# marian42/shapegan

Measured on AMD Instinct MI355X. Metric: GAN train steps/sec @32^3 voxels (train_wgan.py 5 critic + 1 generator updates, batch 64/GPU), higher is better.
Workload: dtype f32; 1 GPU; train_wgan.py 32^3 voxel WGAN, fp32, batch=64 synthetic SDF grids (BASELINE configs[1]); global_batch=64, per_gpu_batch=64, parallelism=dp1

## Files before the change

shapegan_amd/csrc/conv3d.hip:

```cpp
#include "mfma_tile.h"
#include <stdlib.h>

#include "conv_common.h"
#include "../../include/shapegan_hip.h"

namespace sg {

struct PatchCtx {
    int base;
    int mask;
    __device__ __forceinline__ void set(const ConvGeom& g, uint32_t pos) {
        int n, od, oh, ow;
        decode_pos(g, pos, n, od, oh, ow);
        const int id0 = 2 * od - 1, ih0 = 2 * oh - 1, iw0 = 2 * ow - 1;
        base = n * g.Cx * g.ID * g.IH * g.IW + (id0 * g.IH + ih0) * g.IW + iw0;
        int m = 0;
#pragma unroll
        for (int t = 0; t < 4; ++t) {
            if ((unsigned)(id0 + t) < (unsigned)g.ID) m |= 1 << t;
            if ((unsigned)(ih0 + t) < (unsigned)g.IH) m |= 1 << (4 + t);
            if ((unsigned)(iw0 + t) < (unsigned)g.IW) m |= 1 << (8 + t);
        }
        mask = m;
    }
// ... 420 lines not shown
struct WgradEpi {
    float* dw;
    long ldw;
    struct Col {
        int j;
    };
    __device__ Col col(int j) const { return Col{j}; }
    __device__ void store(const Col& c, int i, int j, float v) const { dw[(long)i * ldw + c.j] = v; }
};

}

using namespace sg;

extern "C" {

static bool edge_enabled(int which = 7) {
    constexpr int off = SG_NO_EDGE;
    return (off & which) == 0;
}

size_t sg_conv3d_k4s2p1_dgrad_workspace_bytes(int Cout, int Cin) {
    const size_t a = (size_t)8 * Cout * 8 * Cin * sizeof(float), b = halo_dgrad_workspace_bytes(Cin, Cout);
    return a > b ? a : b;
}

size_t sg_conv3d_k4s2p1_dgrad_workspace_bytes_for(int batch, int Cin, int Cout, int OD, int OH, int OW) {
    const size_t a = sg_conv3d_k4s2p1_dgrad_workspace_bytes(Cout, Cin);
    const size_t b = (Cin == 1 && Cout <= 64) ? edge_dgrad_workspace_bytes(batch, OD, OH, OW) : 0;
    return a > b ? a : b;
}

size_t sg_conv3d_k4s2p1_wgrad_workspace_bytes(int batch, int Cin, int Cout, int OD, int OH, int OW) {
    const size_t a = (size_t)16 * Cout * Cin * 64 * sizeof(float);
    const size_t b = (Cin >= 2 && Cout >= 32) ? halo_wgrad_workspace_bytes(batch, Cin, Cout, OD, OH, OW) : 0;
    const size_t c = (Cin == 1 && Cout <= 64) ? edge_wgrad_workspace_bytes(batch, OD, OH, OW) : 0;
    const size_t ab = a > b ? a : b;
    return ab > c ? ab : c;
}

size_t sg_conv3d_k4s2p1_fwd_workspace_bytes(int batch, int Cin, int Cout, int OD, int OH, int OW) {
    const size_t per = (size_t)batch * Cout * OD * OH * OW;
    const size_t tiles = ((size_t)batch * OD * OH * OW + 63) / 64 * ((Cout + 63) / 64);
    const size_t splitk = tiles >= 512 ? 0 : per * 8 * sizeof(float);
    const size_t pack = halo_fwd_workspace_bytes(Cin, Cout);
    const size_t edge = (Cin == 1 && Cout <= 64) ? edge_fwd_workspace_bytes(batch, OD, OH, OW) : 0;
    const size_t sp = (OD == 4 && OH == 4 && OW == 4) ? pack + splitk : (splitk > pack ? splitk : pack);
    return sp > edge ? sp : edge;
}

static int check_sizes(const ConvGeom& g, int batch, const char* who) {
    const long npos = (long)batch * g.O3();
    if (npos >= (1L << 31) || (long)batch * g.Cx * g.I3() >= (1L << 31) || (long)batch * g.Cy * g.O3() >= (1L << 31))
        SG_FAIL(SG_ERR_ARG, "%s: tensors of 2^31 elements or more are not supported (32-bit gather offsets)", who);
    return 0;
}

}

static int fwd_call(const float* x, const float* w, const float* bias, float* y, int batch, int Cin, int Cin_total,
                    int Cx, int Cout, int ID, int IH, int IW, int act, float slope, void* workspace,
                    size_t workspace_bytes, hipStream_t stream, bool packed_already) {
    SG_CHECK_ARG(x && w && y && batch > 0 && Cin > 0 && Cin <= Cin_total && Cin <= Cx && Cout > 0);
    ConvGeom g;
    if (make_geom(g, ID, IH, IW, Cx, Cout)) SG_FAIL(SG_ERR_ARG, "sg_conv3d_k4s2p1_fwd: spatial dims must be even and >= 2");
    if (check_sizes(g, batch, "sg_conv3d_k4s2p1_fwd")) return SG_ERR_ARG;
    const long npos = (long)batch * g.O3();
    if (Cin == 1 && edge_enabled(1) &&
        edge_fwd_try(x, w, bias, y, batch, Cin, Cin_total, g, Cout, act, slope, workspace, workspace_bytes, stream) == 1) {
        SG_CHECK_LAUNCH();
        return SG_OK;
    }
    {
        const int rc = halo_fwd_try(x, w, bias, y, batch, Cin, Cin_total, g, Cout, act, slope, workspace, workspace_bytes,
                                    stream, 0, 0, packed_already);
        if (rc < 0) return rc;
        if (rc == 1) {
            SG_CHECK_LAUNCH();
            return SG_OK;
        }
        if (rc > 16) {
            const int csplit = rc - 16;
            FwdEpi epi{y, bias, g.O3(), Cout, FastDiv((uint32_t)g.O3()), act, slope};
            const float* partial = reinterpret_cast<const float*>(static_cast<const char*>(workspace) + halo_fwd_workspace_bytes(Cin, Cout));
            const long fb = (long)Cout * ((npos + 1023) >> 10);
            hipLaunchKernelGGL((splitk_finalize_kernel<FwdEpi>), dim3((unsigned)fb), dim3(256), 0, stream, partial, epi, Cout, (int)npos,
                               csplit);
            SG_CHECK_LAUNCH();
            return SG_OK;
        }
    }
    MatRowMajor la;
    la.p = w;
    la.ld = (long)Cin_total * 64;
    FwdPatchLoader lb;
    lb.x = x;
    lb.g = g;
    FwdEpi epi{y, bias, g.O3(), Cout, FastDiv((uint32_t)g.O3()), act, slope};
    size_t ws_use = workspace ? workspace_bytes : 0;
    const size_t ws_query = sg_conv3d_k4s2p1_fwd_workspace_bytes(batch, Cin, Cout, g.OD, g.OH, g.OW);
    if (ws_use > ws_query) ws_use = ws_query;
    launch_tile_gemm(la, lb, epi, Cout, (int)npos, Cin * 64, (float*)workspace, ws_use, stream);
    SG_CHECK_LAUNCH();
    return SG_OK;
}

extern "C" {

int sg_conv3d_k4s2p1_fwd(const float* x, const float* w, const float* bias, float* y, int batch, int Cin, int Cin_total,
                         int Cx, int Cout, int ID, int IH, int IW, int act, float slope, void* workspace,
                         size_t workspace_bytes, hipStream_t stream) {
    return fwd_call(x, w, bias, y, batch, Cin, Cin_total, Cx, Cout, ID, IH, IW, act, slope, workspace, workspace_bytes, stream, false);
}
int sg_conv3d_k4s2p1_fwd_keep(const float* x, const float* w, const float* bias, float* y, int batch, int Cin, int Cin_total,
                              int Cx, int Cout, int ID, int IH, int IW, int act, float slope, void* workspace,
                              size_t workspace_bytes, int weights_unchanged, hipStream_t stream) {
    return fwd_call(x, w, bias, y, batch, Cin, Cin_total, Cx, Cout, ID, IH, IW, act, slope, workspace, workspace_bytes, stream,
                    weights_unchanged != 0);
}

int sg_conv3d_k4s2p1_fwd_impl(const float* x, const float* w, const float* bias, float* y, int batch, int Cin,
                              int Cin_total, int Cx, int Cout, int ID, int IH, int IW, int act, float slope,
                              void* workspace, size_t workspace_bytes, int impl, int debug, hipStream_t stream) {
    SG_CHECK_ARG(x && w && y && batch > 0 && Cin > 0 && Cin <= Cin_total && Cin <= Cx && Cout > 0);
    ConvGeom g;
    if (make_geom(g, ID, IH, IW, Cx, Cout)) SG_FAIL(SG_ERR_ARG, "sg_conv3d_k4s2p1_fwd_impl: bad spatial dims");
    if (check_sizes(g, batch, "sg_conv3d_k4s2p1_fwd_impl")) return SG_ERR_ARG;
    if (impl == 1) {
        const int rc = halo_fwd_try(x, w, bias, y, batch, Cin, Cin_total, g, Cout, act, slope, workspace, workspace_bytes,
                                    stream, 1, debug);
        if (rc != 1) SG_FAIL(SG_ERR_ARG, "sg_conv3d_k4s2p1_fwd_impl: shape not eligible for the LDS-halo kernel");
        SG_CHECK_LAUNCH();
        return SG_OK;
    }
    const long npos = (long)batch * g.O3();
    MatRowMajor la;
    la.p = w;
    la.ld = (long)Cin_total * 64;
    FwdPatchLoader lb;
    lb.x = x;
    lb.g = g;
    FwdEpi epi{y, bias, g.O3(), Cout, FastDiv((uint32_t)g.O3()), act, slope};
    launch_tile_gemm(la, lb, epi, Cout, (int)npos, Cin * 64, (float*)workspace, workspace ? workspace_bytes : 0, stream);
    SG_CHECK_LAUNCH();
    return SG_OK;
}

}

static int dgrad_call(const float* dy, const float* w, const float* bias, float* dx, int batch, int Cin, int Cin_total, int Cx,
                      int Cout, int ID, int IH, int IW, int act, float slope, void* workspace, size_t workspace_bytes,
                      hipStream_t stream, bool packed_already) {
    SG_CHECK_ARG(dy && w && dx && batch > 0 && Cin > 0 && Cin <= Cin_total && Cin <= Cx && Cout > 0);
    ConvGeom g;
    if (make_geom(g, ID, IH, IW, Cx, Cout)) SG_FAIL(SG_ERR_ARG, "sg_conv3d_k4s2p1_dgrad: spatial dims must be even and >= 2");
    if (check_sizes(g, batch, "sg_conv3d_k4s2p1_dgrad")) return SG_ERR_ARG;
    const long npos = (long)batch * g.O3();
    if (Cin == 1 && edge_enabled(2) &&
        edge_dgrad_try(dy, w, bias, dx, batch, Cin, Cin_total, g, Cout, act, slope, workspace, workspace_bytes, stream) == 1) {
        SG_CHECK_LAUNCH();
        return SG_OK;
    }
    if (Cin == 1 && g.OD % kO1D == 0 && g.OH % kO1H == 0 && g.OW % kO1W == 0 && (long)g.Cy * g.O3() * 4 < (long)kBufRange) {
        const int ntd = g.OD / kO1D, nth = g.OH / kO1H, ntw = g.OW / kO1W;
        const size_t lds = (size_t)(2 * kO1CC * (kO1CH + 8) + 8) * sizeof(float);
        static SgPerDeviceOnce attr_once;
        if (attr_once.begin()) {
            (void)hipFuncSetAttribute(reinterpret_cast<const void*>(dgrad_out1_tile_kernel),
                                      hipFuncAttributeMaxDynamicSharedMemorySize, (int)lds);
            attr_once.end();
        }
        hipLaunchKernelGGL(dgrad_out1_tile_kernel, dim3((unsigned)((long)batch * ntd * nth * ntw)), dim3(256), lds, stream, dy, w,
                           bias, dx, g, Cout, Cin_total, ntd, nth, ntw, act, slope);
        SG_CHECK_LAUNCH();
        return SG_OK;
    }
    if (Cin == 1 && Cout <= 512) {
        hipLaunchKernelGGL(dgrad_out1_kernel, dim3((unsigned)((npos + 255) / 256)), dim3(256),
                           (size_t)Cout * 64 * sizeof(float), stream, dy, w, bias, dx, g, Cout, Cin_total, (int)npos, act,
                           slope);
        SG_CHECK_LAUNCH();
        return SG_OK;
    }
    {
        const int rc = halo_dgrad_try(dy, w, bias, dx, batch, Cin, Cin_total, g, Cout, act, slope, workspace,
                                      workspace_bytes, stream, 0, packed_already);
        if (rc < 0) return rc;
        if (rc == 1) {
            SG_CHECK_LAUNCH();
            return SG_OK;
        }
    }
    const size_t need = (size_t)8 * Cout * 8 * Cin * sizeof(float);
    if (!workspace || workspace_bytes < need)
        SG_FAIL(SG_ERR_WORKSPACE, "sg_conv3d_k4s2p1_dgrad: workspace too small (%zu < %zu)", workspace_bytes, need);
    float* wt = (float*)workspace;
    if (!packed_already) {
        const long total = 8L * Cout * 8 * Cin;
        int blocks = (int)((total + 255) / 256);
        if (blocks > 2048) blocks = 2048;
        hipLaunchKernelGGL(pack_dgrad_weights_kernel, dim3(blocks), dim3(256), 0, stream, w, wt, Cout, Cin_total, Cin);
    }
    DgradWeightLoader la;
    la.wt = wt;
    la.Cin = Cin;
    la.pstride = (long)Cout * 8 * Cin;
    DgradPatchLoader lb;
    lb.dy = dy;
    lb.g = g;
    DgradEpi epi{dx, bias, g, act, slope};
    const int M = Cin, N = (int)npos, K = Cout * 8;
    const TilePlan p = plan_tiles(M, N, K, 0, 8);
    dim3 grid(sg_cdiv(N, 64 * p.tn), sg_cdiv(M, 64 * p.tm), 8);
#define SG_DGRAD_LAUNCH(TM_, TN_)                                                                                     \
    hipLaunchKernelGGL((tile_gemm_kernel<TM_, TN_, DgradWeightLoader, DgradPatchLoader, DgradEpi>), grid, dim3(256), 0, \
                       stream, la, lb, epi, M, N, K, 0)
    if (p.tm == 2 && p.tn == 2)
        SG_DGRAD_LAUNCH(2, 2);
    else if (p.tm == 2)
        SG_DGRAD_LAUNCH(2, 1);
    else if (p.tn == 2)
        SG_DGRAD_LAUNCH(1, 2);
    else
        SG_DGRAD_LAUNCH(1, 1);
#undef SG_DGRAD_LAUNCH
    SG_CHECK_LAUNCH();
    return SG_OK;
}

extern "C" {

int sg_conv3d_k4s2p1_dgrad(const float* dy, const float* w, const float* bias, float* dx, int batch, int Cin,
                           int Cin_total, int Cx, int Cout, int ID, int IH, int IW, int act, float slope,
                           void* workspace, size_t workspace_bytes, hipStream_t stream) {
    return dgrad_call(dy, w, bias, dx, batch, Cin, Cin_total, Cx, Cout, ID, IH, IW, act, slope, workspace, workspace_bytes, stream,
                      false);
}
int sg_conv3d_k4s2p1_dgrad_keep(const float* dy, const float* w, const float* bias, float* dx, int batch, int Cin,
                                int Cin_total, int Cx, int Cout, int ID, int IH, int IW, int act, float slope,
                                void* workspace, size_t workspace_bytes, int weights_unchanged, hipStream_t stream) {
    return dgrad_call(dy, w, bias, dx, batch, Cin, Cin_total, Cx, Cout, ID, IH, IW, act, slope, workspace, workspace_bytes, stream,
                      weights_unchanged != 0);
}

int sg_conv3d_k4s2p1_pack_images(int n, const int* kinds, const float* const* weights, void* const* workspaces,
                                 const size_t* workspace_bytes, const int* dims, int* served, hipStream_t stream) {
    SG_CHECK_ARG(n > 0 && n <= 8 && kinds && weights && workspaces && workspace_bytes && dims && served);
    PackJobs jobs;
    static const float dummy = 0.f;
    for (int i = 0; i < n; ++i) {
        const int* d = dims + 8 * i;
        const int batch = d[0], Cin = d[1], Cin_total = d[2], Cx = d[3], Cout = d[4];
        served[i] = 0;
        SG_CHECK_ARG(weights[i] && batch > 0 && Cin > 0 && Cin <= Cin_total && Cin <= Cx && Cout > 0 && (kinds[i] == 0 || kinds[i] == 1));
        ConvGeom g;
        if (make_geom(g, d[5], d[6], d[7], Cx, Cout)) SG_FAIL(SG_ERR_ARG, "sg_conv3d_k4s2p1_pack_images: bad spatial dims");
        if (check_sizes(g, batch, "sg_conv3d_k4s2p1_pack_images")) return SG_ERR_ARG;
        if (Cin == 1) continue;
        int rc;
        if (kinds[i] == 0)
            rc = halo_fwd_try(&dummy, weights[i], nullptr, const_cast<float*>(&dummy), batch, Cin, Cin_total, g, Cout, SG_ACT_NONE, 0.f,
                              workspaces[i], workspace_bytes[i], stream, 0, 0, false, &jobs);
        else
            rc = halo_dgrad_try(&dummy, weights[i], nullptr, const_cast<float*>(&dummy), batch, Cin, Cin_total, g, Cout, SG_ACT_NONE, 0.f,
                                workspaces[i], workspace_bytes[i], stream, 0, false, &jobs);
        if (rc < 0) return rc;
        served[i] = rc == 1;
    }
    halo_pack_jobs_launch(jobs, stream);
    SG_CHECK_LAUNCH();
    return SG_OK;
}

long long sg_conv3d_k4s2p1_image_layout(int kind, const int* dims, size_t workspace_bytes) {
    if (!dims || (kind != 0 && kind != 1)) return 0;
    const int batch = dims[0], Cin = dims[1], Cin_total = dims[2], Cx = dims[3], Cout = dims[4];
    if (batch <= 0 || Cin <= 1 || Cin > Cin_total || Cin > Cx || Cout <= 0) return 0;
    ConvGeom g;
    if (make_geom(g, dims[5], dims[6], dims[7], Cx, Cout)) return 0;
    if ((long)batch * g.O3() >= (1L << 31) || (long)batch * g.I3() >= (1L << 31)) return 0;
    PackJobs jobs;
    static const float dummy = 0.f;
    char* const base = reinterpret_cast<char*>(uintptr_t(1) << 20);
    const int rc = kind == 0 ? halo_fwd_try(&dummy, &dummy, nullptr, const_cast<float*>(&dummy), batch, Cin, Cin_total, g, Cout, SG_ACT_NONE,
                                            0.f, base, workspace_bytes, nullptr, 0, 0, false, &jobs)
                             : halo_dgrad_try(&dummy, &dummy, nullptr, const_cast<float*>(&dummy), batch, Cin, Cin_total, g, Cout,
                                              SG_ACT_NONE, 0.f, base, workspace_bytes, nullptr, 0, false, &jobs);
    if (rc != 1 || jobs.n != 1) return 0;
    const PackJob& j = jobs.job[0];
    unsigned long long h = 1469598103934665603ull;
    const long long f[7] = {j.kind + 1, j.Cout, j.Cin_total, j.Cin, j.nt, (long long)(reinterpret_cast<char*>(j.wp) - base), 0x5347};
    for (long long v : f)
        for (int b = 0; b < 8; ++b) {
            h ^= (unsigned long long)(v >> (8 * b)) & 0xffull;
            h *= 1099511628211ull;
        }
    h &= 0x7fffffffffffffffull;
    return h ? (long long)h : 1;
}

int sg_conv3d_k4s2p1_dgrad_impl(const float* dy, const float* w, const float* bias, float* dx, int batch, int Cin,
                                int Cin_total, int Cx, int Cout, int ID, int IH, int IW, int act, float slope,
                                void* workspace, size_t workspace_bytes, int impl, hipStream_t stream) {
    SG_CHECK_ARG(dy && w && dx && batch > 0 && Cin > 0 && Cin <= Cin_total && Cin <= Cx && Cout > 0 && (impl & 1) &&
                 (impl == 1 || impl == 3 || impl == 9 || impl == 17 || impl == 33));
    ConvGeom g;
    if (make_geom(g, ID, IH, IW, Cx, Cout)) SG_FAIL(SG_ERR_ARG, "sg_conv3d_k4s2p1_dgrad_impl: bad spatial dims");
    if (check_sizes(g, batch, "sg_conv3d_k4s2p1_dgrad_impl")) return SG_ERR_ARG;
    const int rc = halo_dgrad_try(dy, w, bias, dx, batch, Cin, Cin_total, g, Cout, act, slope, workspace, workspace_bytes,
                                  stream, impl);
    if (rc != 1) SG_FAIL(SG_ERR_ARG, "sg_conv3d_k4s2p1_dgrad_impl: shape not eligible for the LDS-halo kernel");
    SG_CHECK_LAUNCH();
    return SG_OK;
}

int sg_conv3d_k4s2p1_wgrad_impl(const float* dy, const float* x, float* dw, int batch, int Cin, int Cin_total, int Cx,
                                int Cout, int ID, int IH, int IW, void* workspace, size_t workspace_bytes, int impl,
                                hipStream_t stream) {
    SG_CHECK_ARG(dy && x && dw && batch > 0 && Cin > 0 && Cin <= Cin_total && Cin <= Cx && Cout > 0 && impl == 1);
    ConvGeom g;
    if (make_geom(g, ID, IH, IW, Cx, Cout)) SG_FAIL(SG_ERR_ARG, "sg_conv3d_k4s2p1_wgrad_impl: bad spatial dims");
    if (check_sizes(g, batch, "sg_conv3d_k4s2p1_wgrad_impl")) return SG_ERR_ARG;
    const int rc = halo_wgrad_try(dy, x, dw, batch, Cin, Cin_total, g, Cout, workspace, workspace_bytes, stream, 1);
    if (rc != 1) SG_FAIL(SG_ERR_ARG, "sg_conv3d_k4s2p1_wgrad_impl: shape not eligible for the LDS-halo kernel");
    SG_CHECK_LAUNCH();
    return SG_OK;
}

int sg_conv3d_k4s2p1_wgrad_dy_image(int batch, int Cin, int Cout, int OD, int OH, int OW, size_t workspace_bytes, int* mt_total,
                                    long* nslice) {
    if (batch <= 0 || Cin <= 0 || Cout <= 0 || !mt_total || !nslice) return 0;
    ConvGeom g;
    if (make_geom(g, 2 * OD, 2 * OH, 2 * OW, Cin, Cout)) return 0;
    if (Cin == 1 && Cout <= 64) return 0;
    return halo_wgrad_dy_image_plan(batch, Cin, Cout, g, workspace_bytes, mt_total, nslice);
}
int sg_act_bwd_rowsum_pack8(const float* y, const float* dy, float* dz, float* rowsum, void* dz_image, long N, int C, long nslice,
                            int act, float slope, hipStream_t stream) {
    SG_CHECK_ARG(y && dy && dz && rowsum && dz_image && N > 0 && C > 0 && C % 128 == 0 && nslice == N * 8);
    SG_CHECK_ARG(act == SG_ACT_LEAKY || act == SG_ACT_RELU);
    SG_CHECK_ARG((((uintptr_t)y | (uintptr_t)dy | (uintptr_t)dz | (uintptr_t)dz_image) & 15) == 0);
    halo_act_bwd_pack8_launch(y, dy, dz, rowsum, dz_image, N * C, C, nslice, act, slope, stream);
    SG_CHECK_LAUNCH();
    return SG_OK;
}
int sg_conv3d_k4s2p1_wgrad_prepacked(const float* dy, const float* x, float* dw, int batch, int Cin, int Cin_total, int Cx,
                                     int Cout, int ID, int IH, int IW, void* workspace, size_t workspace_bytes, hipStream_t stream) {
    SG_CHECK_ARG(dy && x && dw && batch > 0 && Cin > 0 && Cin <= Cin_total && Cin <= Cx && Cout > 0);
    ConvGeom g;
    if (make_geom(g, ID, IH, IW, Cx, Cout)) SG_FAIL(SG_ERR_ARG, "sg_conv3d_k4s2p1_wgrad_prepacked: bad spatial dims");
    if (check_sizes(g, batch, "sg_conv3d_k4s2p1_wgrad_prepacked")) return SG_ERR_ARG;
    int mt;
    long ns;
    if (!halo_wgrad_dy_image_plan(batch, Cin, Cout, g, workspace_bytes, &mt, &ns))
        SG_FAIL(SG_ERR_ARG, "sg_conv3d_k4s2p1_wgrad_prepacked: this call is not served with a producer-written image");
    if (halo_wgrad_try(dy, x, dw, batch, Cin, Cin_total, g, Cout, workspace, workspace_bytes, stream, 0, true) != 1)
        SG_FAIL(SG_ERR_ARG, "sg_conv3d_k4s2p1_wgrad_prepacked: not served");
    SG_CHECK_LAUNCH();
    return SG_OK;
}

int sg_conv3d_k4s2p1_wgrad_act_eligible(int batch, int Cin, int Cout, int OD, int OH, int OW, int act) {
    const size_t x_bytes = ((size_t)batch * 8 * OD * OH * OW + (size_t)(2 * OH + 1) * 2 * OW + 4) * 4;
    const size_t dy_bytes = (size_t)batch * Cout * OD * OH * OW * 4;
    return Cin == 1 && Cout <= 64 && OW % 16 == 0 && (long)batch * OD * OH * OW >= 65536 && (act == SG_ACT_LEAKY || act == SG_ACT_RELU) &&
           x_bytes < (size_t)kBufRange && dy_bytes < (size_t)kBufRange && edge_enabled(4);
}
int sg_conv3d_k4s2p1_wgrad_act(const float* dy, const float* y, const float* x, float* dw, float* db, int batch, int Cin,
                               int Cin_total, int Cx, int Cout, int ID, int IH, int IW, int act, float slope, void* workspace,
                               size_t workspace_bytes, hipStream_t stream) {
    SG_CHECK_ARG(dy && y && x && dw && db && batch > 0 && Cin > 0 && Cin <= Cin_total && Cin <= Cx && Cout > 0);
    ConvGeom g;
    if (make_geom(g, ID, IH, IW, Cx, Cout)) SG_FAIL(SG_ERR_ARG, "sg_conv3d_k4s2p1_wgrad_act: spatial dims must be even and >= 2");
    if (check_sizes(g, batch, "sg_conv3d_k4s2p1_wgrad_act")) return SG_ERR_ARG;
    if (!sg_conv3d_k4s2p1_wgrad_act_eligible(batch, Cin, Cout, g.OD, g.OH, g.OW, act) ||
        edge_wgrad_try(dy, x, dw, batch, Cin, Cin_total, g, Cout, workspace, workspace ? workspace_bytes : 0, stream, 0, y, act, slope,
                       db) != 1)
        SG_FAIL(SG_ERR_ARG, "sg_conv3d_k4s2p1_wgrad_act: shape not served (see sg_conv3d_k4s2p1_wgrad_act_eligible) or workspace too small");
    SG_CHECK_LAUNCH();
    return SG_OK;
}

int sg_conv3d_k4s2p1_wgrad(const float* dy, const float* x, float* dw, int batch, int Cin, int Cin_total, int Cx,
                           int Cout, int ID, int IH, int IW, void* workspace, size_t workspace_bytes,
                           hipStream_t stream) {
    SG_CHECK_ARG(dy && x && dw && batch > 0 && Cin > 0 && Cin <= Cin_total && Cin <= Cx && Cout > 0);
    ConvGeom g;
    if (make_geom(g, ID, IH, IW, Cx, Cout)) SG_FAIL(SG_ERR_ARG, "sg_conv3d_k4s2p1_wgrad: spatial dims must be even and >= 2");
    if (check_sizes(g, batch, "sg_conv3d_k4s2p1_wgrad")) return SG_ERR_ARG;
    const long npos = (long)batch * g.O3();
    if (Cin == 1 && edge_enabled(4) &&
        edge_wgrad_try(dy, x, dw, batch, Cin, Cin_total, g, Cout, workspace, workspace ? workspace_bytes : 0, stream) == 1) {
        SG_CHECK_LAUNCH();
        return SG_OK;
    }
    {
        const int rc = halo_wgrad_try(dy, x, dw, batch, Cin, Cin_total, g, Cout, workspace, workspace ? workspace_bytes : 0,
                                      stream, 0);
        if (rc < 0) return rc;
        if (rc == 1) {
            SG_CHECK_LAUNCH();
            return SG_OK;
        }
    }
    WgradDyLoader la;
    la.dy = dy;
    la.O3 = (int)g.O3();
    la.Cy = Cout;
    la.dO3 = FastDiv((uint32_t)g.O3());
    WgradPatchLoader lb;
    lb.x = x;
    lb.g = g;
    WgradEpi epi{dw, (long)Cin_total * 64};
    launch_tile_gemm(la, lb, epi, Cout, Cin * 64, (int)npos, (float*)workspace, workspace ? workspace_bytes : 0, stream);
    SG_CHECK_LAUNCH();
    return SG_OK;
}

int sg_convT3d_k4s2p1_fwd(const float* x, const float* w, const float* bias, float* y, int batch, int Cin_T, int Cout_T,
                          int ID, int IH, int IW, int act, float slope, void* workspace, size_t workspace_bytes,
                          hipStream_t stream) {
    return sg_conv3d_k4s2p1_dgrad(x, w, bias, y, batch, Cout_T, Cout_T, Cout_T, Cin_T, 2 * ID, 2 * IH, 2 * IW, act,
                                  slope, workspace, workspace_bytes, stream);
}
int sg_convT3d_k4s2p1_to1_pre_eligible(int batch, int C, int ID, int IH, int IW) {
    return batch > 0 && C > 0 && C <= 64 && ID > 0 && IH > 0 && IW > 0 && IH * IW <= 256 &&
           (size_t)C * ID * IH * IW * 4 < (size_t)kBufRange && (long)batch * 8 * ID * IH * IW < (1L << 31);
}
static int convT_to1_pre(const float* x, const float* w, const float* bias, float* y, const float* in_scale,
                         const float* in_shift, int in_act, float in_slope, int batch, int C, int ID, int IH, int IW,
                         int act, float slope, int samples_per_group, long y_group_stride, int form, hipStream_t stream) {
    SG_CHECK_ARG(x && w && y && in_scale && in_shift && samples_per_group > 0 && batch % samples_per_group == 0 && form >= 0 && form <= 8);
    SG_CHECK_ARG(y_group_stride >= (long)samples_per_group * 8 * ID * IH * IW);
    if (!sg_convT3d_k4s2p1_to1_pre_eligible(batch, C, ID, IH, IW))
        SG_FAIL(SG_ERR_ARG, "sg_convT3d_k4s2p1_to1_pre: shape not served (C <= 64, IH * IW <= 256)");
    SG_CHECK_ARG(in_act == SG_ACT_NONE || in_act == SG_ACT_RELU || (in_act == SG_ACT_LEAKY && in_slope >= 0.f && in_slope <= 1.f));
    ConvGeom g;
    if (make_geom(g, 2 * ID, 2 * IH, 2 * IW, 1, C)) SG_FAIL(SG_ERR_ARG, "sg_convT3d_k4s2p1_to1_pre: bad spatial dims");
    if (edge_dgrad_stream_try(x, w, bias, y, batch, 1, 1, g, C, act, slope, stream, in_scale, in_shift, in_act, in_slope,
                              samples_per_group, y_group_stride, form) != 1)
        SG_FAIL(SG_ERR_ARG, "sg_convT3d_k4s2p1_to1_pre: not served");
    SG_CHECK_LAUNCH();
    return SG_OK;
}
int sg_convT3d_k4s2p1_to1_pre_grouped(const float* x, const float* w, const float* bias, float* y, const float* in_scale,
                                      const float* in_shift, int in_act, float in_slope, int batch, int C, int ID, int IH, int IW,
                                      int act, float slope, int samples_per_group, long y_group_stride, hipStream_t stream) {
    return convT_to1_pre(x, w, bias, y, in_scale, in_shift, in_act, in_slope, batch, C, ID, IH, IW, act, slope, samples_per_group,
                         y_group_stride, 0, stream);
}
int sg_convT3d_k4s2p1_to1_pre_impl(const float* x, const float* w, const float* bias, float* y, const float* in_scale,
                                   const float* in_shift, int in_act, float in_slope, int batch, int C, int ID, int IH, int IW,
                                   int act, float slope, int form, hipStream_t stream) {
    return convT_to1_pre(x, w, bias, y, in_scale, in_shift, in_act, in_slope, batch, C, ID, IH, IW, act, slope, batch,
                         (long)batch * 8 * ID * IH * IW, form, stream);
}
int sg_convT3d_k4s2p1_to1_pre(const float* x, const float* w, const float* bias, float* y, const float* in_scale,
                              const float* in_shift, int in_act, float in_slope, int batch, int C, int ID, int IH, int IW, int act,
                              float slope, hipStream_t stream) {
    return sg_convT3d_k4s2p1_to1_pre_grouped(x, w, bias, y, in_scale, in_shift, in_act, in_slope, batch, C, ID, IH, IW, act, slope,
                                             batch, (long)batch * 8 * ID * IH * IW, stream);
}
int sg_convT3d_k4s2p1_dgrad(const float* dy, const float* w, float* dx, int batch, int Cin_T, int Cout_T, int ID, int IH,
                            int IW, void* workspace, size_t workspace_bytes, hipStream_t stream) {
    return sg_conv3d_k4s2p1_fwd(dy, w, nullptr, dx, batch, Cout_T, Cout_T, Cout_T, Cin_T, 2 * ID, 2 * IH, 2 * IW,
                                SG_ACT_NONE, 0.f, workspace, workspace_bytes, stream);
}
int sg_convT3d_k4s2p1_wgrad(const float* dy, const float* x, float* dw, int batch, int Cin_T, int Cout_T, int ID, int IH,
                            int IW, void* workspace, size_t workspace_bytes, hipStream_t stream) {
    return sg_conv3d_k4s2p1_wgrad(x, dy, dw, batch, Cout_T, Cout_T, Cout_T, Cin_T, 2 * ID, 2 * IH, 2 * IW, workspace,
                                  workspace_bytes, stream);
}

}
```

shapegan_amd/csrc/conv3d_halo.hip:

```cpp
#include "conv_common.h"

#ifndef SG_RING
#define SG_RING 8
#endif
#ifndef SG_ABLATE
#define SG_ABLATE 0
#endif

namespace sg {

constexpr int kHD = 4, kHH = 18, kHWF = 18;
constexpr int kHWH = 10;
constexpr int kROWH = 2 * kHWH;
constexpr int kROWD = kHH * kROWH;
constexpr int kHS = kHD * kROWD;
constexpr int kCC = 4;

struct HaloFwdArgs {
    const float* x;
    const float4* wp;
    const float* bias;
    float* y;
    ConvGeom g;
    int Cin, Cout;
    int nth, ntw;
    FastDiv dntw, dnth, dOD;
    int act;
    float slope;
    int csplit;
    float* partial;
    long npos;
};

__global__ void __launch_bounds__(256) pack_fwd_weights_kernel(const float* __restrict__ w, float4* __restrict__ wp,
                                                               int Cout, int Cin_total, int Cin, int ntile) {
    const long G = (long)Cin * 8;
    const long total = (long)ntile * G * 64;
    for (long e = (long)blockIdx.x * 256 + threadIdx.x; e < total; e += (long)gridDim.x * 256) {
        const int lane = (int)(e & 63);
        const long q = e >> 6;
        const long g = q % G;
        const int mt = (int)(q / G);
        const int co = mt * 32 + (lane & 31);
        float4 v = make_float4(0.f, 0.f, 0.f, 0.f);
        if (co < Cout) {
            const float* src = w + (long)co * Cin_total * 64 + g * 8 + (lane >> 5);
            v = make_float4(src[0], src[2], src[4], src[6]);
        }
        wp[e] = v;
    }
}

template <int TN, int NW>
__global__ void __launch_bounds__(NW * 64) conv_fwd_halo_kernel(HaloFwdArgs a) {
    constexpr int kFR = NW * 2;
    constexpr int kNF = (kHD * kHH + kFR - 1) / kFR;
    constexpr int WN = 2 / TN;
    constexpr int ROWS = (NW / WN) * 32;
    constexpr int kRing = SG_RING;
    constexpr int kBUF = kCC * kHS;
    extern __shared__ __attribute__((aligned(16))) float halo[];
    lds_float* const hl = (lds_float*)halo;

    uint32_t twi, thi, od, n, q1, q2;
    a.dntw.divmod(blockIdx.x, q1, twi);
    a.dnth.divmod(q1, q2, thi);
    a.dOD.divmod(q2, n, od);
    const int oh0 = thi * 8, ow0 = twi * 8;
    const int co0 = blockIdx.y * ROWS;

    const int tid = threadIdx.x, lane = tid & 63;
    const int wave = __builtin_amdgcn_readfirstlane(tid >> 6);
    const int wm = wave / WN, wn = wave % WN, r = lane & 31, kpar = lane >> 5;
    const int lanebase = 2 * (wn * TN * 4 + (r >> 3)) * kROWH + kpar * kHWH + (r & 7);
    constexpr int kTNOFF = 2 * 4 * kROWH;

    f32x16 acc[TN];
#pragma unroll
    for (int u = 0; u < TN; ++u)
#pragma unroll
        for (int q = 0; q < 16; ++q) acc[u][q] = 0.f;

    const lds_float* bb[2][kCC][4];
#pragma unroll
    for (int b = 0; b < 2; ++b)
#pragma unroll
        for (int c = 0; c < kCC; ++c)
#pragma unroll
            for (int kd = 0; kd < 4; ++kd) {
                bb[b][c][kd] = hl + b * kBUF + c * kHS + kd * kROWD + lanebase;
                pin_vgpr(bb[b][c][kd]);
            }

    const int G = a.Cin * 8;
    const __amdgpu_buffer_rsrc_t wres = make_rsrc(a.wp + ((long)(co0 / 32 + wm) * G) * 64);
    const unsigned wvoff = lane * 16;

    const int I3 = a.g.ID * a.g.IH * a.g.IW;
    const __amdgpu_buffer_rsrc_t xres = make_rsrc(a.x + (long)n * a.g.Cx * I3);
    const int fl_w = tid & 31, frow = tid >> 5;
    const int iw = 2 * ow0 - 1 + fl_w;
    const bool wok = fl_w < kHWF && (unsigned)iw < (unsigned)a.g.IW;
    const int lds_w = (fl_w & 1) * kHWH + (fl_w >> 1);
    const int pad = (tid % (kHD * kHH * 2)) * kHWH + (kHWH - 1);
    unsigned goff[kNF];
    lds_float* sdst[kNF];
#pragma unroll
    for (int f = 0; f < kNF; ++f) {
        const int row = kFR * f + frow, hd = row / kHH, hh = row - hd * kHH;
        const int id = 2 * (int)od - 1 + hd, ih = 2 * oh0 - 1 + hh;
        const bool inbox = fl_w < kHWF && row < kHD * kHH;
        const bool ok = inbox && wok && (unsigned)id < (unsigned)a.g.ID && (unsigned)ih < (unsigned)a.g.IH;
        goff[f] = ok ? (unsigned)((id * a.g.IH + ih) * a.g.IW + iw) * 4u : kBufOutside;
        sdst[f] = hl + (inbox ? hd * kROWD + hh * kROWH + lds_w : pad);
        pin_vgpr(goff[f]);
        pin_vgpr(sdst[f]);
    }
    float fv[kCC][kNF];
    const unsigned chan_bytes = (unsigned)I3 * 4u;

#pragma unroll
    for (int c = 0; c < kCC; ++c)
#pragma unroll
        for (int f = 0; f < kNF; ++f) fv[c][f] = buf_load(xres, goff[f], c * chan_bytes);
    float4 aring[kRing];
#pragma unroll
    for (int u = 0; u < kRing; ++u) aring[u] = buf_load4(wres, wvoff, (unsigned)(u < G ? u : G - 1) * 1024u);
#pragma unroll
    for (int c = 0; c < kCC; ++c)
#pragma unroll
        for (int f = 0; f < kNF; ++f) sdst[f][c * kHS] = fv[c][f];
    __syncthreads();

    const int nstage = a.Cin / kCC;
    int gbase = kRing;

    auto stage = [&](auto tag, int s) {
        constexpr int CUR = decltype(tag)::value, NXT = CUR ^ 1;
        int cnext = (s + 1) * kCC;
        cnext = cnext > a.Cin - kCC ? a.Cin - kCC : cnext;
        const unsigned xs = (unsigned)cnext * chan_bytes;
        float bq[TN][4];
#pragma unroll
        for (int u = 0; u < TN; ++u) {
            const lds_float* hb = bb[CUR][0][0] + u * kTNOFF;
            bq[u][0] = hb[0];
            bq[u][1] = hb[1];
            bq[u][2] = hb[kROWH];
            bq[u][3] = hb[kROWH + 1];
        }
        __builtin_amdgcn_sched_barrier(0);
#pragma unroll
        for (int ci = 0; ci < kCC; ++ci) {
#pragma unroll
            for (int j = 0; j < 8; ++j) {
                const float4 a_cur = aring[(ci * 8 + j) % kRing];
                int gi = gbase + ci * 8 + j;
                gi = gi < G ? gi : G - 1;
                if (!(SG_ABLATE & 4)) aring[(ci * 8 + j) % kRing] = buf_load4(wres, wvoff, (unsigned)gi * 1024u);
                {
                    constexpr int NE = kCC * kNF;
                    const int gidx = ci * 8 + j;
#pragma unroll
                    for (int e = 0; e < NE; ++e) {
                        const int c = e / kNF, f = e % kNF;
                        if (e * 24 / NE + 8 == gidx && !(SG_ABLATE & 2)) sdst[f][NXT * kBUF + c * kHS] = fv[c][f];
                        if (e * 24 / NE == gidx && !(SG_ABLATE & 3)) fv[c][f] = buf_load(xres, goff[f], xs + c * chan_bytes);
                    }
                }
                float b[TN][4];
#pragma unroll
                for (int u = 0; u < TN; ++u)
#pragma unroll
                    for (int k = 0; k < 4; ++k) b[u][k] = bq[u][k];
                if (!(ci == kCC - 1 && j == 7) && !(SG_ABLATE & 16)) {
                    const int jn = (j + 1) & 7, cin = ci + ((j + 1) >> 3);
                    const lds_float* hb = bb[CUR][cin][jn >> 1] + (2 * (jn & 1)) * kROWH;
#pragma unroll
                    for (int u = 0; u < TN; ++u) {
                        bq[u][0] = hb[u * kTNOFF];
                        bq[u][1] = hb[u * kTNOFF + 1];
                        bq[u][2] = hb[u * kTNOFF + kROWH];
                        bq[u][3] = hb[u * kTNOFF + kROWH + 1];
                    }
                }
                __builtin_amdgcn_sched_barrier(0);
#pragma unroll
                for (int k = 0; k < 4; ++k)
#pragma unroll
                    for (int u = 0; u < TN; ++u) {
                        const float av = k == 0 ? a_cur.x : (k == 1 ? a_cur.y : (k == 2 ? a_cur.z : a_cur.w));
                        acc[u] = __builtin_amdgcn_mfma_f32_32x32x2f32(av, b[u][k], acc[u], 0, 0, 0);
                    }
                __builtin_amdgcn_sched_barrier(0);
            }
        }
        gbase += 8 * kCC;
        __syncthreads();
    };
    for (int s = 0; s + 1 < nstage; s += 2) {
        stage(IntTag<0>(), s);
        stage(IntTag<1>(), s + 1);
    }
    if (nstage & 1) stage(IntTag<0>(), nstage - 1);

    const long O3 = (long)a.g.OD * a.g.OH * a.g.OW;
    float bv[16];
#pragma unroll
    for (int q = 0; q < 16; ++q) {
        const int co = co0 + wm * 32 + (q & 3) + 8 * (q >> 2) + 4 * kpar;
        bv[q] = a.bias ? a.bias[co < a.Cout ? co : a.Cout - 1] : 0.f;
    }
#pragma unroll
    for (int u = 0; u < TN; ++u) {
        const int ph = (wn * TN + u) * 4 + (r >> 3), pw = r & 7;
        float* yo = a.y + (long)n * a.Cout * O3 + ((long)od * a.g.OH + (oh0 + ph)) * a.g.OW + (ow0 + pw);
#pragma unroll
        for (int q = 0; q < 16; ++q) {
            const int co = co0 + wm * 32 + (q & 3) + 8 * (q >> 2) + 4 * kpar;
            if (co < a.Cout) yo[(long)co * O3] = sg_apply_act(acc[u][q] + bv[q], a.act, a.slope);
        }
    }
}

constexpr int k4HALF = 5, k4ROW = 10, k4PLANE = 104, k4CH = 10 * k4PLANE;
constexpr int k4CC = 8;
constexpr int k4BUF = k4CC * k4CH;

__global__ void __launch_bounds__(512) conv_fwd_halo4_kernel(HaloFwdArgs a) {
    constexpr int kRing = 8;
    extern __shared__ __attribute__((aligned(16))) float halo[];
    lds_float* const hl = (lds_float*)halo;
    const int n = blockIdx.x, co0 = blockIdx.y * 64;
    const int cpw = a.Cin / a.csplit, cb = blockIdx.z * cpw;
    const int tid = threadIdx.x, lane = tid & 63;
    const int wave = __builtin_amdgcn_readfirstlane(tid >> 6);
    const int kh = wave >> 2, wm = (wave >> 1) & 1, wn = wave & 1, r = lane & 31, kpar = lane >> 5;
    const int p = wn * 32 + r, od = p >> 4, oh = (p >> 2) & 3, ow = p & 3;
    const int lanebase = 2 * od * k4PLANE + 2 * oh * k4ROW + kpar * k4HALF + ow;

    f32x16 acc;
#pragma unroll
    for (int q = 0; q < 16; ++q) acc[q] = 0.f;

    for (int e = tid; e < 2 * k4BUF; e += 512) hl[e] = 0.f;

    const lds_float* bb[2][4][4];
#pragma unroll
    for (int b = 0; b < 2; ++b)
#pragma unroll
        for (int c = 0; c < 4; ++c)
#pragma unroll
            for (int kd = 0; kd < 4; ++kd) {
                bb[b][c][kd] = hl + b * k4BUF + (kh * 4 + c) * k4CH + kd * k4PLANE + lanebase;
                pin_vgpr(bb[b][c][kd]);
            }
    const int G = a.Cin * 8;
    const __amdgpu_buffer_rsrc_t wres = make_rsrc(a.wp + ((long)(co0 / 32 + wm) * G) * 64);
    const unsigned wvoff = lane * 16;

    const int I3 = 512;
    const __amdgpu_buffer_rsrc_t xres = make_rsrc(a.x + ((long)n * a.g.Cx + cb) * I3);
    unsigned xvoff = tid * 4;
    lds_float* sdst = hl + ((tid >> 6) + 1) * k4PLANE + (((tid >> 3) & 7) + 1) * k4ROW + (((tid & 7) + 1) & 1) * k4HALF +
                      (((tid & 7) + 1) >> 1);
    pin_vgpr(xvoff);
    pin_vgpr(sdst);
    float fv[k4CC];
    __syncthreads();
#pragma unroll
    for (int c = 0; c < k4CC; ++c) fv[c] = buf_load(xres, xvoff, c * (I3 * 4));
    const int nstage = cpw / k4CC, nq = nstage * 32, s0 = cb / k4CC;
    auto group_of = [&](int q) {
        q = q < nq ? q : nq - 1;
        return ((q >> 5) + s0) * 64 + kh * 32 + (q & 31);
    };
    float4 aring[kRing];
#pragma unroll
    for (int u = 0; u < kRing; ++u) aring[u] = buf_load4(wres, wvoff, (unsigned)group_of(u) * 1024u);
#pragma unroll
    for (int c = 0; c < k4CC; ++c) sdst[c * k4CH] = fv[c];
    __syncthreads();

    int qbase = kRing;
    auto stage = [&](auto tag, int s) {
        constexpr int CUR = decltype(tag)::value, NXT = CUR ^ 1;
        int cnext = (s + 1) * k4CC;
        cnext = cnext > cpw - k4CC ? cpw - k4CC : cnext;
        const unsigned xs = (unsigned)cnext * (I3 * 4);
        float bq[4];
        {
            const lds_float* hb = bb[CUR][0][0];
            bq[0] = hb[0];
            bq[1] = hb[1];
            bq[2] = hb[k4ROW];
            bq[3] = hb[k4ROW + 1];
        }
        __builtin_amdgcn_sched_barrier(0);
#pragma unroll
        for (int ci = 0; ci < 4; ++ci) {
#pragma unroll
            for (int j = 0; j < 8; ++j) {
                const int gidx = ci * 8 + j;
                const float4 a_cur = aring[gidx % kRing];
                aring[gidx % kRing] = buf_load4(wres, wvoff, (unsigned)group_of(qbase + gidx) * 1024u);
#pragma unroll
                for (int c = 0; c < k4CC; ++c) {
                    if (2 * c + 8 == gidx) sdst[NXT * k4BUF + c * k4CH] = fv[c];
                    if (2 * c == gidx) fv[c] = buf_load(xres, xvoff, xs + c * (I3 * 4));
                }
                float b[4];
#pragma unroll
                for (int k = 0; k < 4; ++k) b[k] = bq[k];
                if (gidx + 1 < 32) {
                    const int jn = (j + 1) & 7, cin = ci + ((j + 1) >> 3);
                    const lds_float* hb = bb[CUR][cin][jn >> 1] + (2 * (jn & 1)) * k4ROW;
                    bq[0] = hb[0];
                    bq[1] = hb[1];
                    bq[2] = hb[k4ROW];
                    bq[3] = hb[k4ROW + 1];
                }
                __builtin_amdgcn_sched_barrier(0);
                acc = __builtin_amdgcn_mfma_f32_32x32x2f32(a_cur.x, b[0], acc, 0, 0, 0);
                acc = __builtin_amdgcn_mfma_f32_32x32x2f32(a_cur.y, b[1], acc, 0, 0, 0);
                acc = __builtin_amdgcn_mfma_f32_32x32x2f32(a_cur.z, b[2], acc, 0, 0, 0);
                acc = __builtin_amdgcn_mfma_f32_32x32x2f32(a_cur.w, b[3], acc, 0, 0, 0);
                __builtin_amdgcn_sched_barrier(0);
            }
        }
        qbase += 32;
        __syncthreads();
    };
    for (int s = 0; s + 1 < nstage; s += 2) {
        stage(IntTag<0>(), s);
        stage(IntTag<1>(), s + 1);
    }
    if (nstage & 1) stage(IntTag<0>(), nstage - 1);

    float* red = halo + ((wave & 3) * 16) * 64;
    if (kh == 1) {
#pragma unroll
        for (int q = 0; q < 16; ++q) red[q * 64 + lane] = acc[q];
    }
    __syncthreads();
    if (kh == 1) return;
    if (a.csplit > 1) {
        float* po = a.partial + (long)blockIdx.z * a.Cout * a.npos + (long)n * 64 + p;
#pragma unroll
        for (int q = 0; q < 16; ++q) {
            const int co = co0 + wm * 32 + (q & 3) + 8 * (q >> 2) + 4 * kpar;
            if (co < a.Cout) po[(long)co * a.npos] = acc[q] + red[q * 64 + lane];
        }
        return;
    }
    float* yo = a.y + (long)n * a.Cout * 64 + p;
#pragma unroll
    for (int q = 0; q < 16; ++q) {
        const int co = co0 + wm * 32 + (q & 3) + 8 * (q >> 2) + 4 * kpar;
        if (co < a.Cout) {
            const float bv = a.bias ? a.bias[co] : 0.f;
            yo[(long)co * 64] = sg_apply_act(acc[q] + red[q * 64 + lane] + bv, a.act, a.slope);
        }
    }
}

size_t halo_fwd_workspace_bytes(int Cin, int Cout) { return (size_t)((Cout + 127) / 128) * 128 * Cin * 64 * sizeof(float); }

int halo_fwd_try(const float* x, const float* w, const float* bias, float* y, int batch, int Cin, int Cin_total,
                 const ConvGeom& g, int Cout, int act, float slope, void* workspace, size_t workspace_bytes,
                 hipStream_t stream, int force, int debug, bool packed_already, PackJobs* collect) {
    if (g.OD == 4 && g.OH == 4 && g.OW == 4) {
        if (Cin % k4CC != 0 || Cin < 2 * k4CC || Cout < 32) return 0;
        if (!workspace || workspace_bytes < halo_fwd_workspace_bytes(Cin, Cout)) return 0;
        if ((long)g.Cx * 512 * 4 >= (long)kBufRange || (long)Cin * 8 * 1024 >= (long)kBufRange || batch > 65535 * 16) return 0;
        const int mtiles = sg_cdiv(Cout, 64);
        int csplit = 1;
        if (!force && (long)batch * mtiles < 160) {
            while (csplit < 8 && (long)batch * mtiles * csplit < 256 && (Cin / (2 * csplit)) % k4CC == 0 && Cin / (2 * csplit) >= 2 * k4CC)
                csplit *= 2;
            if (csplit == 1) return 0;
            if (workspace_bytes < halo_fwd_workspace_bytes(Cin, Cout) + (size_t)csplit * Cout * batch * 64 * sizeof(float)) return 0;
        }
        float4* wp = (float4*)workspace;
        const int ntile = mtiles * 2;
        const long total = (long)ntile * Cin * 8 * 64;
        int blocks = (int)((total + 255) / 256);
        if (blocks > 4096) blocks = 4096;
        if (collect) return collect->add(0, w, wp, Cout, Cin_total, Cin, ntile);
        if (!packed_already)
            hipLaunchKernelGGL(pack_fwd_weights_kernel, dim3(blocks), dim3(256), 0, stream, w, wp, Cout, Cin_total, Cin, ntile);
        HaloFwdArgs a;
        a.x = x;
        a.wp = wp;
        a.bias = bias;
        a.y = y;
        a.g = g;
        a.Cin = Cin;
        a.Cout = Cout;
        a.nth = a.ntw = 1;
        a.dntw = a.dnth = a.dOD = FastDiv(1);
        a.act = act;
        a.slope = slope;
        a.csplit = csplit;
        a.partial = reinterpret_cast<float*>(static_cast<char*>(workspace) + halo_fwd_workspace_bytes(Cin, Cout));
        a.npos = (long)batch * 64;
        const size_t lds4 = (size_t)2 * k4BUF * sizeof(float);
        static SgPerDeviceOnce attr_once;
        if (attr_once.begin()) {
            (void)hipFuncSetAttribute(reinterpret_cast<const void*>(conv_fwd_halo4_kernel),
                                      hipFuncAttributeMaxDynamicSharedMemorySize, (int)lds4);
            attr_once.end();
        }
        hipLaunchKernelGGL(conv_fwd_halo4_kernel, dim3((unsigned)batch, mtiles, csplit), dim3(512), lds4, stream, a);
        return csplit > 1 ? 16 + csplit : 1;
    }
    if (g.OW % 8 != 0 || g.OH % 8 != 0 || Cin % kCC != 0 || Cin < 8 || Cout < 32) return 0;
    if ((long)g.Cx * g.ID * g.IH * g.IW * 4 >= (long)kBufRange || (long)Cin * 8 * 1024 >= (long)kBufRange) return 0;
    if (!workspace || workspace_bytes < halo_fwd_workspace_bytes(Cin, Cout)) return 0;
    if ((long)batch * g.Cx * g.ID * g.IH * g.IW >= (1L << 31)) return 0;
    int variant = (debug >> 4) & 3;
    int rows = (Cout > 64 && ((debug >> 4) & 3) != 3) ? 128 : 64;
    const int ntw = g.OW / 8, nth = g.OH / 8;
    const long tiles = (long)batch * g.OD * nth * ntw;
    if (rows == 128 && variant == 0 && !(debug & 128)) {
        const long w128 = tiles * sg_cdiv(Cout, 128);
        if (w128 <= 128 || (w128 > 256 && w128 <= 384)) rows = 64;
    }
    const int mtiles = sg_cdiv(Cout, rows);
    if (!force && tiles * mtiles < (rows == 128 ? 144 : 192)) return 0;
    if (tiles >= (1L << 31)) return 0;
    if (variant == 0) variant = 2;
    size_t lds = (size_t)2 * kCC * kHS * sizeof(float);
    if (tiles * mtiles < 256 * 3 * 4 && !(debug & 64) && lds < 56 * 1024) lds = 56 * 1024;

    float4* wp = (float4*)workspace;
    {
        const int ntile = mtiles * rows / 32;
        const long total = (long)ntile * Cin * 8 * 64;
        int blocks = (int)((total + 255) / 256);
        if (blocks > 4096) blocks = 4096;
        if (collect) return collect->add(0, w, wp, Cout, Cin_total, Cin, ntile);
        if (!packed_already)
            hipLaunchKernelGGL(pack_fwd_weights_kernel, dim3(blocks), dim3(256), 0, stream, w, wp, Cout, Cin_total, Cin, ntile);
    }
    HaloFwdArgs a;
    a.x = x;
    a.wp = wp;
    a.bias = bias;
    a.y = y;
    a.g = g;
    a.Cin = Cin;
    a.Cout = Cout;
    a.nth = nth;
    a.ntw = ntw;
    a.dntw = FastDiv(ntw);
    a.dnth = FastDiv(nth);
    a.dOD = FastDiv(g.OD);
    a.act = act;
    a.slope = slope;
    dim3 grid((unsigned)tiles, mtiles);
    if (rows == 128 && variant == 2)
        hipLaunchKernelGGL((conv_fwd_halo_kernel<1, 8>), grid, dim3(512), lds, stream, a);
    else if (rows == 128)
        hipLaunchKernelGGL((conv_fwd_halo_kernel<2, 4>), grid, dim3(256), lds, stream, a);
    else
        hipLaunchKernelGGL((conv_fwd_halo_kernel<1, 4>), grid, dim3(256), lds, stream, a);
    return 1;
}


template <int MODE>
struct DBox;
template <>
struct DBox<0> {
    static constexpr int BH = 9, BW = 9, PL = 81, CH = 243, TNOFF = 36, WNOFF = 81;
};
template <>
struct DBox<1> {
    static constexpr int BH = 5, BW = 5, PL = 25, CH = 250, TNOFF = 50, WNOFF = 125;
};

struct HaloDgradArgs {
    const float* dy;
    const float4* wp;
    const float* bias;
    float* dx;
    ConvGeom g;
    int Cin, Cout, mtiles, batch;
    int ppw;
    FastDiv dntw, dnth, dntd;
    int act;
    float slope;
};

__global__ void __launch_bounds__(256) pack_dgrad_frag_kernel(const float* __restrict__ w, float4* __restrict__ wp,
                                                              int Cout, int Cin_total, int Cin, int MT) {
    const long total = 8L * MT * Cout * 64;
    for (long e = (long)blockIdx.x * 256 + threadIdx.x; e < total; e += (long)gridDim.x * 256) {
        const int lane = (int)(e & 63);
        long q = e >> 6;
        const int co = (int)(q % Cout);
        q /= Cout;
        const int mt = (int)(q % MT);
        const int p = (int)(q / MT);
        const int ci = mt * 32 + (lane & 31);
        float v[4] = {0.f, 0.f, 0.f, 0.f};
        if (ci < Cin) {
            const float* src = w + ((long)co * Cin_total + ci) * 64;
#pragma unroll
            for (int j = 0; j < 4; ++j) {
                const int t = 2 * j + (lane >> 5);
                const int kd = 1 - ((p >> 2) & 1) + 2 * ((t >> 2) & 1);
                const int kh = 1 - ((p >> 1) & 1) + 2 * ((t >> 1) & 1);
                const int kw = 1 - (p & 1) + 2 * (t & 1);
                v[j] = src[kd * 16 + kh * 4 + kw];
            }
        }
        wp[e] = make_float4(v[0], v[1], v[2], v[3]);
    }
}

__global__ void __launch_bounds__(256) pack_images_kernel(PackJobs jobs) {
    const PackJob& j = jobs.job[blockIdx.y];
    float4* __restrict__ wp = j.wp;
    const float* __restrict__ w = j.w;
    if (j.kind == 0) {
        const long G = (long)j.Cin * 8;
        const long total = (long)j.nt * G * 64;
        for (long e = (long)blockIdx.x * 256 + threadIdx.x; e < total; e += (long)gridDim.x * 256) {
            const int lane = (int)(e & 63);
            const long q = e >> 6;
            const long g = q % G;
            const int mt = (int)(q / G);
            const int co = mt * 32 + (lane & 31);
            float4 v = make_float4(0.f, 0.f, 0.f, 0.f);
            if (co < j.Cout) {
                const float* src = w + (long)co * j.Cin_total * 64 + g * 8 + (lane >> 5);
                v = make_float4(src[0], src[2], src[4], src[6]);
            }
            wp[e] = v;
        }
    } else {
        const int MT = j.nt;
        const long total = 8L * MT * j.Cout * 64;
        for (long e = (long)blockIdx.x * 256 + threadIdx.x; e < total; e += (long)gridDim.x * 256) {
            const int lane = (int)(e & 63);
            long q = e >> 6;
            const int co = (int)(q % j.Cout);
            q /= j.Cout;
            const int mt = (int)(q % MT);
            const int p = (int)(q / MT);
            const int ci = mt * 32 + (lane & 31);
            float v[4] = {0.f, 0.f, 0.f, 0.f};
            if (ci < j.Cin) {
                const float* src = w + ((long)co * j.Cin_total + ci) * 64;
#pragma unroll
                for (int jj = 0; jj < 4; ++jj) {
                    const int t = 2 * jj + (lane >> 5);
                    const int kd = 1 - ((p >> 2) & 1) + 2 * ((t >> 2) & 1);
                    const int kh = 1 - ((p >> 1) & 1) + 2 * ((t >> 1) & 1);
                    const int kw = 1 - (p & 1) + 2 * (t & 1);
                    v[jj] = src[kd * 16 + kh * 4 + kw];
                }
            }
            wp[e] = make_float4(v[0], v[1], v[2], v[3]);
        }
    }
}
int halo_pack_jobs_launch(const PackJobs& jobs, hipStream_t stream) {
    if (jobs.n <= 0) return 0;
    hipLaunchKernelGGL(pack_images_kernel, dim3(1024, jobs.n), dim3(256), 0, stream, jobs);
    return jobs.n;
}

template <int MODE, bool R32>
__device__ __forceinline__ void conv_dgrad_halo_body(HaloDgradArgs a) {
    constexpr int NTN = R32 ? 1 : 2;
    constexpr int kDCC = 16, kDNF = 16, kDBUF = kDNF * 256;
    using BX = DBox<MODE>;
    constexpr int kDB = BX::CH;
    extern __shared__ __attribute__((aligned(16))) float box[];
    uint32_t twi = 0, thi = 0, tdi = 0, n, q1, q2;
    if (MODE == 0) {
        a.dntw.divmod(blockIdx.x, q1, twi);
        a.dnth.divmod(q1, q2, thi);
        a.dntd.divmod(q2, n, tdi);
    } else {
        n = blockIdx.x * 2;
    }
    const int qd0 = tdi * 2, qh0 = thi * 8, qw0 = twi * 8;
    const int ci0 = blockIdx.y * (R32 ? 32 : 64);

    const int tid = threadIdx.x, lane = tid & 63;
    const int wave = __builtin_amdgcn_readfirstlane(tid >> 6);
    const int wm = R32 ? 0 : wave >> 1, wn = wave & 1, r = lane & 31, kpar = lane >> 5;
    const int tnf = R32 ? wave >> 1 : 0;
    const int lpart = MODE == 0 ? (r >> 3) * BX::BW + (r & 7) : (r >> 4) * BX::PL + ((r >> 2) & 3) * BX::BW + (r & 3);
    const int lanebase = wn * BX::WNOFF + tnf * BX::TNOFF + lpart + 1 - kpar;

    f32x16 acc[NTN];
#pragma unroll
    for (int t = 0; t < NTN; ++t)
#pragma unroll
        for (int q = 0; q < 16; ++q) acc[t][q] = 0.f;

    lds_float* const bl = (lds_float*)box;
    const lds_float* bb[2][kDCC];
#pragma unroll
    for (int b = 0; b < 2; ++b)
#pragma unroll
        for (int c = 0; c < kDCC; ++c) {
            bb[b][c] = bl + b * kDBUF + c * kDB + lanebase;
            pin_vgpr(bb[b][c]);
        }
    lds_float* sdst = bl + tid;
    pin_vgpr(sdst);

    const int G = a.Cout;
    const int par0 = blockIdx.z * a.ppw, par_end = par0 + a.ppw;
    const unsigned par_bytes = (unsigned)(a.mtiles * 2) * (unsigned)G * 1024u;
    const __amdgpu_buffer_rsrc_t wres = make_rsrc(a.wp + ((long)(R32 ? blockIdx.y : blockIdx.y * 2 + wm) * G) * 64);
    const unsigned wvoff = lane * 16;

    const int O3 = a.g.OD * a.g.OH * a.g.OW;
    const int obias = (a.g.OH + 1) * a.g.OW + 1;
    const __amdgpu_buffer_rsrc_t dres = __builtin_amdgcn_make_buffer_rsrc(
        const_cast<float*>(a.dy + (long)n * a.g.Cy * O3 - obias), 0, 1 << 26, 0x00020000);
    const unsigned chan_bytes = (unsigned)O3 * 4u;
    unsigned gword[kDNF], goff[kDNF];
#pragma unroll
    for (int f = 0; f < kDNF; ++f) {
        const int e = tid + 256 * f;
        const int ci = e / kDB;
        int rem = e - ci * kDB, smp = 0;
        if (MODE == 1) {
            smp = rem / 125;
            rem -= smp * 125;
        }
        const int hd = rem / BX::PL, hh = (rem - hd * BX::PL) / BX::BW, hw = rem % BX::BW;
        const int od = qd0 - 1 + hd, oh = qh0 - 1 + hh, ow = qw0 - 1 + hw;
        const bool never = e >= kDCC * kDB || (int)n + smp >= a.batch;
        const unsigned cls = (od < 0 ? 1u << 26 : 0u) | (od + 1 >= a.g.OD ? 1u << 27 : 0u) | (oh < 0 ? 1u << 28 : 0u) |
                             (oh + 1 >= a.g.OH ? 1u << 29 : 0u) | (ow < 0 ? 1u << 30 : 0u) | (ow + 1 >= a.g.OW ? 1u << 31 : 0u);
        const int off0 = (smp * a.g.Cy + ci) * O3 + (od * a.g.OH + oh) * a.g.OW + ow + obias;
        gword[f] = never ? 0xffffffffu : ((unsigned)off0 * 4u) | cls;
        pin_vgpr(gword[f]);
    }
    unsigned pshift = 0;
    auto set_goff = [&](int par) __attribute__((always_inline)) {
        const int pd = (par >> 2) & 1, ph = (par >> 1) & 1, pw = par & 1;
        const unsigned mask = 0x03ffffffu | (pd ? 1u << 27 : 1u << 26) | (ph ? 1u << 29 : 1u << 28) | (pw ? 1u << 31 : 1u << 30);
#pragma unroll
        for (int f = 0; f < kDNF; ++f) goff[f] = gword[f] & mask;
        pshift = (unsigned)((pd * a.g.OH + ph) * a.g.OW + pw) * 4u;
    };
    const long I3 = (long)a.g.ID * a.g.IH * a.g.IW;
    const int nn = MODE == 0 ? (int)n : (int)n + wn;
    const __amdgpu_buffer_rsrc_t ores = make_rsrc(a.dx + (long)(nn < a.batch ? nn : 0) * a.g.Cx * I3);
    const __amdgpu_buffer_rsrc_t bres = make_rsrc(a.bias ? a.bias : a.dx);
    unsigned ovoff[NTN];
#pragma unroll
    for (int tn = 0; tn < NTN; ++tn) {
        int qd, qh, qw;
        if (MODE == 0) {
            qd = qd0 + wn;
            qh = qh0 + (tnf + tn) * 4 + (r >> 3);
            qw = qw0 + (r & 7);
        } else {
            qd = 2 * (tnf + tn) + (r >> 4);
            qh = (r >> 2) & 3;
            qw = r & 3;
        }
        ovoff[tn] = (unsigned)(((2 * qd) * a.g.IH + 2 * qh) * a.g.IW + 2 * qw + 4 * kpar * (int)I3) * 4u;
        pin_vgpr(ovoff[tn]);
    }
    const unsigned bvoff = kpar * 16;
#ifdef SG_DGRAD_NO_PAIR
    const bool paired = false;
#else
    const bool paired = a.ppw >= 2;
#endif
    float keep[NTN][16];
#pragma unroll
    for (int t = 0; t < NTN; ++t)
#pragma unroll
        for (int q = 0; q < 16; ++q) keep[t][q] = 0.f;
    auto write_parity = [&](int par) __attribute__((always_inline)) {
        const int pd = (par >> 2) & 1, ph = (par >> 1) & 1, pw = par & 1;
        const unsigned oshift = (unsigned)((pd * a.g.IH + ph) * a.g.IW) * 4u;
        if (nn < a.batch) {
            if (paired && pw == 0) {
#pragma unroll
                for (int q = 0; q < 16; ++q) {
                    const int cis = ci0 + wm * 32 + (q & 3) + 8 * (q >> 2);
                    const float bv = a.bias && cis < a.Cin ? buf_load(bres, bvoff, (unsigned)cis * 4u) : 0.f;
#pragma unroll
                    for (int tn = 0; tn < NTN; ++tn) keep[tn][q] = sg_apply_act(acc[tn][q] + bv, a.act, a.slope);
                }
            } else if (paired) {
                typedef unsigned u32x2 __attribute__((ext_vector_type(2)));
#pragma unroll
                for (int q = 0; q < 16; ++q) {
                    const int cis = ci0 + wm * 32 + (q & 3) + 8 * (q >> 2);
                    if (cis < a.Cin) {
                        const float bv = a.bias ? buf_load(bres, bvoff, (unsigned)cis * 4u) : 0.f;
#pragma unroll
                        for (int tn = 0; tn < NTN; ++tn) {
                            u32x2 v;
                            v.x = __builtin_bit_cast(unsigned, keep[tn][q]);
                            v.y = __builtin_bit_cast(unsigned, sg_apply_act(acc[tn][q] + bv, a.act, a.slope));
                            __builtin_amdgcn_raw_buffer_store_b64(v, ores, (int)ovoff[tn], (int)((unsigned)cis * (unsigned)I3 * 4u + oshift), 0);
                        }
                    }
                }
            } else {
#pragma unroll
                for (int q = 0; q < 16; ++q) {
                    const int cis = ci0 + wm * 32 + (q & 3) + 8 * (q >> 2);
                    if (cis < a.Cin) {
                        const float bv = a.bias ? buf_load(bres, bvoff, (unsigned)cis * 4u) : 0.f;
#pragma unroll
                        for (int tn = 0; tn < NTN; ++tn) {
                            const float v = sg_apply_act(acc[tn][q] + bv, a.act, a.slope);
                            __builtin_amdgcn_raw_buffer_store_b32(__builtin_bit_cast(unsigned, v), ores, (int)ovoff[tn],
                                                                  (int)((unsigned)cis * (unsigned)I3 * 4u + oshift + 4u * pw), 0);
                        }
                    }
                }
            }
        }
#pragma unroll
        for (int t = 0; t < NTN; ++t)
#pragma unroll
            for (int q = 0; q < 16; ++q) acc[t][q] = 0.f;
    };

    set_goff(par0);
    float fv[kDNF];
    constexpr int kRing = 8;
    float4 aring[kRing];
    unsigned wcur = (unsigned)par0 * par_bytes;
#pragma unroll
    for (int f = 0; f < kDNF; ++f) fv[f] = buf_load(dres, goff[f], pshift);
#pragma unroll
    for (int u = 0; u < kRing; ++u) aring[u] = buf_load4(wres, wvoff, wcur + (unsigned)u * 1024u);
#pragma unroll
    for (int f = 0; f < kDNF; ++f) sdst[256 * f] = fv[f];
    __syncthreads();

    constexpr int O00 = BX::PL + BX::BW, O01 = BX::PL, O10 = BX::BW, O11 = 0;
    const int nstage = a.Cout / kDCC;
    auto stage = [&](auto tag, unsigned dys, unsigned wnext) __attribute__((always_inline)) {
        constexpr int CUR = decltype(tag)::value, NXT = CUR ^ 1;
        float bq[NTN][4];
#pragma unroll
        for (int tn = 0; tn < NTN; ++tn) {
            const lds_float* hb = bb[CUR][0] + tn * BX::TNOFF;
            bq[tn][0] = hb[O00];
            bq[tn][1] = hb[O01];
            bq[tn][2] = hb[O10];
            bq[tn][3] = hb[O11];
        }
        __builtin_amdgcn_sched_barrier(0);
#pragma unroll
        for (int c = 0; c < kDCC; ++c) {
            const float4 a_cur = aring[c % kRing];
            aring[c % kRing] = c + kRing < kDCC ? buf_load4(wres, wvoff, wcur + (unsigned)(c + kRing) * 1024u)
                                                : buf_load4(wres, wvoff, wnext + (unsigned)(c + kRing - kDCC) * 1024u);
            float b[NTN][4];
#pragma unroll
            for (int tn = 0; tn < NTN; ++tn)
#pragma unroll
                for (int j = 0; j < 4; ++j) b[tn][j] = bq[tn][j];
            if (c + 1 < kDCC) {
#pragma unroll
                for (int tn = 0; tn < NTN; ++tn) {
                    const lds_float* hb = bb[CUR][c + 1] + tn * BX::TNOFF;
                    bq[tn][0] = hb[O00];
                    bq[tn][1] = hb[O01];
                    bq[tn][2] = hb[O10];
                    bq[tn][3] = hb[O11];
                }
            }
            if (c < kDCC / 2) {
#pragma unroll
                for (int f = 2 * c; f < 2 * c + 2; ++f) fv[f] = buf_load(dres, goff[f], dys + pshift);
            } else {
#pragma unroll
                for (int f = 2 * (c - kDCC / 2); f < 2 * (c - kDCC / 2) + 2; ++f) sdst[NXT * kDBUF + 256 * f] = fv[f];
            }
            __builtin_amdgcn_sched_barrier(0);
            const float av[4] = {a_cur.x, a_cur.y, a_cur.z, a_cur.w};
#pragma unroll
            for (int j = 0; j < 4; ++j)
#pragma unroll
                for (int tn = 0; tn < NTN; ++tn) acc[tn] = __builtin_amdgcn_mfma_f32_32x32x2f32(av[j], b[tn][j], acc[tn], 0, 0, 0);
            __builtin_amdgcn_sched_barrier(0);
        }
        wcur = wnext;
        __syncthreads();
    };
    for (int par = par0; par < par_end; ++par) {
        const bool more = par + 1 < par_end;
        const unsigned wlast = more ? (unsigned)(par + 1) * par_bytes : (unsigned)par * par_bytes + (unsigned)(nstage - 1) * kDCC * 1024u;
        const unsigned dlast = more ? 0u : (unsigned)(nstage - 1) * kDCC * chan_bytes;
        int s = 0;
        for (; s + 1 < nstage; s += 2) {
            stage(IntTag<0>(), (unsigned)(s + 1) * kDCC * chan_bytes, wcur + kDCC * 1024u);
            const bool last = s + 2 == nstage;
            if (last && more) set_goff(par + 1);
            stage(IntTag<1>(), last ? dlast : (unsigned)(s + 2) * kDCC * chan_bytes, last ? wlast : wcur + kDCC * 1024u);
        }
        if (s < nstage) stage(IntTag<0>(), dlast, wlast);
        write_parity(par);
    }
}

template <int MODE>
__global__ void __launch_bounds__(256) conv_dgrad_halo_kernel(HaloDgradArgs a) {
    conv_dgrad_halo_body<MODE, false>(a);
}
template <int MODE>
__global__ void __launch_bounds__(256) conv_dgrad_halo32_kernel(HaloDgradArgs a) {
    conv_dgrad_halo_body<MODE, true>(a);
}

size_t halo_dgrad_workspace_bytes(int Cin, int Cout) { return (size_t)8 * ((Cin + 63) / 64) * 64 * Cout * 8 * sizeof(float); }

int halo_dgrad_try(const float* dy, const float* w, const float* bias, float* dx, int batch, int Cin, int Cin_total,
                   const ConvGeom& g, int Cout, int act, float slope, void* workspace, size_t workspace_bytes,
                   hipStream_t stream, int force, bool packed_already, PackJobs* collect) {
    const bool mode1 = g.OD == 4 && g.OH == 4 && g.OW == 4;
    if (!mode1 && (g.OW % 8 != 0 || g.OH % 8 != 0 || g.OD % 2 != 0)) return 0;
    if (Cout % 16 != 0 || Cin < 32 || Cin % 8 != 0) return 0;
    if (((long)2 * g.Cy * g.OD * g.OH * g.OW + (long)(g.OH + 1) * g.OW + 1) * 4 >= (1L << 26)) return 0;
    if (!workspace || workspace_bytes < halo_dgrad_workspace_bytes(Cin, Cout)) return 0;
    if ((long)batch * g.Cy * g.OD * g.OH * g.OW >= (1L << 31)) return 0;
    if ((long)2 * g.Cy * g.OD * g.OH * g.OW * 4 >= (long)kBufRange || (long)Cout * 1024 >= (long)kBufRange) return 0;
    const int ntw = mode1 ? 1 : g.OW / 8, nth = mode1 ? 1 : g.OH / 8, ntd = mode1 ? 1 : g.OD / 2;
    const long tiles = mode1 ? (batch + 1) / 2 : (long)batch * ntd * nth * ntw;
    const int mtiles = (Cin + 63) / 64;
    if (!force && tiles * mtiles * 8 < (mode1 ? 16 : 64)) return 0;
    if (tiles >= (1L << 31) || mtiles > 65535) return 0;
    float4* wp = (float4*)workspace;
    if ((long)8 * mtiles * 2 * Cout * 1024 >= (long)kBufRange) return 0;
    if (collect) return collect->add(1, w, wp, Cout, Cin_total, Cin, mtiles * 2);
    if (!packed_already) {
        const long total = 8L * mtiles * 2 * Cout * 64;
        int blocks = (int)((total + 255) / 256);
        if (blocks > 4096) blocks = 4096;
        hipLaunchKernelGGL(pack_dgrad_frag_kernel, dim3(blocks), dim3(256), 0, stream, w, wp, Cout, Cin_total, Cin, mtiles * 2);
    }
    HaloDgradArgs a;
    a.dy = dy;
    a.wp = wp;
    a.bias = bias;
    a.dx = dx;
    a.g = g;
    a.Cin = Cin;
    a.Cout = Cout;
    a.mtiles = mtiles;
    a.batch = batch;
    a.dntw = FastDiv(ntw);
    a.dnth = FastDiv(nth);
    a.dntd = FastDiv(ntd);
    a.act = act;
    a.slope = slope;
    int ppw = 8;
    while (ppw > 1 && (tiles * mtiles * (8 / ppw) < 512 || (force & 2) || (Cout / 16) % 2 != 0)) ppw >>= 1;
    if ((force >> 2) && (Cout / 16) % 2 == 0) ppw = force >> 2;
    if ((long)8 * mtiles * 2 * Cout * 1024 >= (long)kBufRange) return 0;
    a.ppw = ppw;
    size_t lds = (size_t)2 * 16 * 256 * sizeof(float);
    {
        const long wgs = tiles * mtiles * (8 / ppw);
        const long cost2 = ((wgs + 511) / 512) * 2, cost3 = ((wgs + 767) / 768) * 3;
        if (cost2 <= cost3) lds = 56 * 1024;
    }
    const bool r32 = Cin <= 32 || tiles * mtiles * (8 / ppw) < 256;
    const dim3 grid((unsigned)tiles, r32 ? (unsigned)((Cin + 31) / 32) : (unsigned)mtiles, 8 / ppw);
    if (mode1 && r32)
        hipLaunchKernelGGL((conv_dgrad_halo32_kernel<1>), grid, dim3(256), lds, stream, a);
    else if (mode1)
        hipLaunchKernelGGL((conv_dgrad_halo_kernel<1>), grid, dim3(256), lds, stream, a);
    else if (r32)
        hipLaunchKernelGGL((conv_dgrad_halo32_kernel<0>), grid, dim3(256), lds, stream, a);
    else
        hipLaunchKernelGGL((conv_dgrad_halo_kernel<0>), grid, dim3(256), lds, stream, a);
    return 1;
}

constexpr int kWROWD = 368;
constexpr int kWHS = kHD * kWROWD;
constexpr int kWNF = (2 * kHD * kHH + 7) / 8;

struct HaloWgradArgs {
    const float4* ap;
    const float* x;
    float* ws;
    ConvGeom g;
    int Cin, Cout, nslice, per_split, mt_total;
    long ldw;
    FastDiv dntw, dnth, dOD;
};

__global__ void __launch_bounds__(256) pack_wgrad_dy_kernel(const float* __restrict__ dy, float4* __restrict__ ap,
                                                            ConvGeom g, int Cout, int MT, int nslice, FastDiv dntw,
                                                            FastDiv dnth, FastDiv dOD) {
    const long total = (long)MT * nslice * 8 * 64;
    const long O3 = (long)g.OD * g.OH * g.OW;
    for (long e = (long)blockIdx.x * 256 + threadIdx.x; e < total; e += (long)gridDim.x * 256) {
        const int lane = (int)(e & 63);
        const int gq = (int)((e >> 6) & 7);
        const long q = e >> 9;
        const uint32_t sl = (uint32_t)(q % nslice);
        const int mt = (int)(q / nslice);
        uint32_t twi, thi, od, n, q1, q2;
        dntw.divmod(sl, q1, twi);
        dnth.divmod(q1, q2, thi);
        dOD.divmod(q2, n, od);
        const int co = mt * 32 + (lane & 31);
        float4 v = make_float4(0.f, 0.f, 0.f, 0.f);
        if (co < Cout) {
            const float* src = dy + ((long)n * Cout + co) * O3 + ((long)od * g.OH + (thi * 8 + gq)) * g.OW + twi * 8 + (lane >> 5);
            v = make_float4(src[0], src[2], src[4], src[6]);
        }
        ap[e] = v;
    }
}

template <int NCH>
__global__ void __launch_bounds__(256) conv_wgrad_halo_kernel(HaloWgradArgs a) {
    extern __shared__ __attribute__((aligned(16))) float wbox[];
    const int tid = threadIdx.x, lane = tid & 63;
    const int wave = __builtin_amdgcn_readfirstlane(tid >> 6);
    const int wm = NCH == 2 ? wave >> 1 : 0, wn = NCH == 2 ? wave & 1 : wave, r = lane & 31, kpar = lane >> 5;
    const int ci0 = blockIdx.x * NCH;
    const int mt0 = blockIdx.y * (NCH == 2 ? 4 : 2);
    constexpr int NF = NCH == 2 ? kWNF : 2 * kWNF;
    constexpr int NV = NCH == 2 ? kWNF : kWNF / 2;
    const int split = blockIdx.z;
    const int s_beg = split * a.per_split, s_end = min(a.nslice, s_beg + a.per_split);

    int lanebase[2];
#pragma unroll
    for (int tn = 0; tn < 2; ++tn) {
        const int col = wn * 64 + tn * 32 + r;
        const int tap = col & 63, kd = tap >> 4, kh = (tap >> 2) & 3, kw = tap & 3;
        lanebase[tn] = (col >> 6) * kWHS + kd * kWROWD + kh * kROWH + (kw & 1) * kHWH + (kw >> 1) + kpar;
    }

    f32x16 acc[2][2];
#pragma unroll
    for (int i = 0; i < 2; ++i)
#pragma unroll
        for (int j = 0; j < 2; ++j)
#pragma unroll
            for (int q = 0; q < 16; ++q) acc[i][j][q] = 0.f;

    const int I3 = a.g.ID * a.g.IH * a.g.IW;
    const int fl_w = tid & 31, frow = tid >> 5;
    const int lds_w = (fl_w & 1) * kHWH + (fl_w >> 1);
    const int prow = (tid >> 1) % (kHD * kHH);
    const int pad = (prow / kHH) * kWROWD + (prow % kHH) * kROWH + (tid & 1) * kHWH + (kHWH - 1);
    lds_float* const wl = (lds_float*)wbox;
    lds_float* sdst[kWNF / 2];
    unsigned voff[NV], cls[NV];
#pragma unroll
    for (int f = 0; f < kWNF / 2; ++f) {
        const int row = 8 * f + frow;
        const int hd = row / kHH, hh = row - hd * kHH;
        const bool inbox = fl_w < kHWF && row < kHD * kHH;
        sdst[f] = wl + (inbox ? hd * kWROWD + hh * kROWH + lds_w : pad);
        pin_vgpr(sdst[f]);
#pragma unroll
        for (int c = 0; c < (NCH == 2 ? 2 : 1); ++c) {
            const bool ok = inbox && (ci0 + c) < a.Cin;
            voff[c * (kWNF / 2) + f] = ok ? (unsigned)(c * I3 + (hd * a.g.IH + hh) * a.g.IW + fl_w) * 4u : kBufOutside;
            cls[c * (kWNF / 2) + f] = (hd == 0 ? 1u << 26 : 0u) | (hd == kHD - 1 ? 1u << 27 : 0u) | (hh == 0 ? 1u << 28 : 0u) |
                                      (hh == kHH - 1 ? 1u << 29 : 0u) | (fl_w == 0 ? 1u << 30 : 0u) |
                                      (fl_w == kHWF - 1 ? 1u << 31 : 0u);
            pin_vgpr(voff[c * (kWNF / 2) + f]);
            pin_vgpr(cls[c * (kWNF / 2) + f]);
        }
    }
    float fv[NF];
    unsigned eoff[NV];
    __amdgpu_buffer_rsrc_t xres;
    auto xres_of = [&]() __attribute__((always_inline)) { return xres; };
    const unsigned chan_bytes = (unsigned)I3 * 4u;
    auto copy_load = [&](int f) __attribute__((always_inline)) {
        if constexpr (NCH == 2) {
            return buf_load(xres_of(), eoff[f], 0);
        } else {
            return buf_load(xres_of(), eoff[f % (kWNF / 2)], (unsigned)(f / (kWNF / 2)) * chan_bytes);
        }
    };
    const int ntw_ = (int)a.g.OW / 8, nth_ = (int)a.g.OH / 8;
    auto copy_prepare = [&](int sl) {
        uint32_t twi, thi, od, n, q1, q2;
        a.dntw.divmod((uint32_t)sl, q1, twi);
        a.dnth.divmod(q1, q2, thi);
        a.dOD.divmod(q2, n, od);
        const long origin = ((long)n * a.g.Cx + ci0) * I3 + ((2 * (long)od - 1) * a.g.IH + (16 * (long)thi - 1)) * a.g.IW +
                            (16 * (long)twi - 1);
        xres = __builtin_amdgcn_make_buffer_rsrc(const_cast<float*>(a.x + origin), 0, 1 << 26, 0x00020000);
        const unsigned flags = (od == 0 ? 1u << 26 : 0u) | ((int)od == a.g.OD - 1 ? 1u << 27 : 0u) | (thi == 0 ? 1u << 28 : 0u) |
                               ((int)thi == nth_ - 1 ? 1u << 29 : 0u) | (twi == 0 ? 1u << 30 : 0u) |
                               ((int)twi == ntw_ - 1 ? 1u << 31 : 0u);
#pragma unroll
        for (int f = 0; f < NV; ++f) eoff[f] = (cls[f] & flags) | voff[f];
    };

    const int nst = s_end - s_beg;
    constexpr int kRing = 8;
    const int G = nst * 8;
    if (nst > 0) {
        __amdgpu_buffer_rsrc_t ares[2];
#pragma unroll
        for (int t = 0; t < 2; ++t) ares[t] = make_rsrc(a.ap + ((long)(mt0 + wm * 2 + t) * a.nslice + s_beg) * 8 * 64);
        const unsigned avoff = lane * 16;
        const lds_float* bb[2][2][2];
#pragma unroll
        for (int b = 0; b < 2; ++b)
#pragma unroll
            for (int tn = 0; tn < 2; ++tn)
#pragma unroll
                for (int h = 0; h < 2; ++h) {
                    bb[b][tn][h] = wl + b * (NCH * kWHS) + lanebase[tn] + h * (8 * kROWH);
                    pin_vgpr(bb[b][tn][h]);
                }

        copy_prepare(s_beg);
#pragma unroll
        for (int f = 0; f < NF; ++f) fv[f] = copy_load(f);
        float4 aring[kRing][2];
#pragma unroll
        for (int u = 0; u < kRing; ++u)
#pragma unroll
            for (int t = 0; t < 2; ++t) aring[u][t] = buf_load4(ares[t], avoff, (unsigned)(u < G ? u : G - 1) * 1024u);
#pragma unroll
        for (int f = 0; f < NF; ++f) sdst[f % (kWNF / 2)][(f / (kWNF / 2)) * kWHS] = fv[f];
        __syncthreads();

        auto stage = [&](auto tag, int st) {
            constexpr int CUR = decltype(tag)::value, NXT = CUR ^ 1;
            const int snext = st + 1 < nst ? st + 1 : st;
            float bq[2][4];
#pragma unroll
            for (int tn = 0; tn < 2; ++tn) {
                const lds_float* hb = bb[CUR][tn][0];
                bq[tn][0] = hb[0];
                bq[tn][1] = hb[2];
                bq[tn][2] = hb[4];
                bq[tn][3] = hb[6];
            }
            copy_prepare(s_beg + snext);
            __builtin_amdgcn_sched_barrier(0);
#pragma unroll
            for (int gq = 0; gq < 8; ++gq) {
                float4 a_cur[2];
#pragma unroll
                for (int t = 0; t < 2; ++t) a_cur[t] = aring[gq][t];
                int gi = (st + 1) * 8 + gq;
                gi = gi < G ? gi : G - 1;
#pragma unroll
                for (int t = 0; t < 2; ++t) aring[gq][t] = buf_load4(ares[t], avoff, (unsigned)gi * 1024u);
                float b[2][4];
#pragma unroll
                for (int tn = 0; tn < 2; ++tn)
#pragma unroll
                    for (int j = 0; j < 4; ++j) b[tn][j] = bq[tn][j];
                if (gq + 1 < 8) {
#pragma unroll
                    for (int tn = 0; tn < 2; ++tn) {
                        const lds_float* hb = bb[CUR][tn][(gq + 1) >> 2] + 2 * ((gq + 1) & 3) * kROWH;
                        bq[tn][0] = hb[0];
                        bq[tn][1] = hb[2];
                        bq[tn][2] = hb[4];
                        bq[tn][3] = hb[6];
                    }
                }
#pragma unroll
                for (int f = 0; f < NF; ++f) {
                    if (f * 4 / NF == gq) fv[f] = copy_load(f);
                    if (f * 4 / NF + 4 == gq) sdst[f % (kWNF / 2)][NXT * (NCH * kWHS) + (f / (kWNF / 2)) * kWHS] = fv[f];
                }
                __builtin_amdgcn_sched_barrier(0);
#pragma unroll
                for (int j = 0; j < 4; ++j) {
                    const float a0 = j == 0 ? a_cur[0].x : (j == 1 ? a_cur[0].y : (j == 2 ? a_cur[0].z : a_cur[0].w));
                    const float a1 = j == 0 ? a_cur[1].x : (j == 1 ? a_cur[1].y : (j == 2 ? a_cur[1].z : a_cur[1].w));
                    acc[0][0] = __builtin_amdgcn_mfma_f32_32x32x2f32(a0, b[0][j], acc[0][0], 0, 0, 0);
                    acc[1][0] = __builtin_amdgcn_mfma_f32_32x32x2f32(a1, b[0][j], acc[1][0], 0, 0, 0);
                    acc[0][1] = __builtin_amdgcn_mfma_f32_32x32x2f32(a0, b[1][j], acc[0][1], 0, 0, 0);
                    acc[1][1] = __builtin_amdgcn_mfma_f32_32x32x2f32(a1, b[1][j], acc[1][1], 0, 0, 0);
                }
                __builtin_amdgcn_sched_barrier(0);
            }
            __syncthreads();
        };
        for (int st = 0; st + 1 < nst; st += 2) {
            stage(IntTag<0>(), st);
            stage(IntTag<1>(), st + 1);
        }
        if (nst & 1) stage(IntTag<0>(), nst - 1);
    }

    float* out = a.ws + (long)split * a.Cout * a.ldw;
#pragma unroll
    for (int tn = 0; tn < 2; ++tn) {
        const int col = wn * 64 + tn * 32 + r;
        const int ci = ci0 + (col >> 6);
        if (ci >= a.Cin) continue;
        const long cbase = (long)ci * 64 + (col & 63);
#pragma unroll
        for (int t = 0; t < 2; ++t) {
#pragma unroll
            for (int q = 0; q < 16; ++q) {
                const int co = (mt0 + wm * 2 + t) * 32 + (q & 3) + 8 * (q >> 2) + 4 * kpar;
                if (co < a.Cout) out[(long)co * a.ldw + cbase] = acc[t][tn][q];
            }
        }
    }
}

__global__ void __launch_bounds__(256) pack_wgrad_dy4_kernel(const float* __restrict__ dy, float4* __restrict__ ap, int Cout,
                                                             int MT, int nslice) {
    const long total = (long)MT * nslice * 8 * 64;
    for (long e = (long)blockIdx.x * 256 + threadIdx.x; e < total; e += (long)gridDim.x * 256) {
        const int lane = (int)(e & 63);
        const int gq = (int)((e >> 6) & 7);
        const long q = e >> 9;
        const long sl = q % nslice;
        const int mt = (int)(q / nslice);
        const int co = mt * 32 + (lane & 31);
        float4 v = make_float4(0.f, 0.f, 0.f, 0.f);
        if (co < Cout) {
            const float* src = dy + (sl * Cout + co) * 64 + (gq >> 1) * 16 + (gq & 1) * 8 + (lane >> 5);
            v = make_float4(src[0], src[2], src[4], src[6]);
        }
        ap[e] = v;
    }
}

__global__ void __launch_bounds__(256) conv_wgrad_halo4_kernel(HaloWgradArgs a) {
    constexpr int kBUF = 2 * k4CH;
    extern __shared__ __attribute__((aligned(16))) float wbox[];
    lds_float* const wl = (lds_float*)wbox;
    const int tid = threadIdx.x, lane = tid & 63;
    const int wave = __builtin_amdgcn_readfirstlane(tid >> 6);
    const int wm = wave >> 1, wn = wave & 1, r = lane & 31, kpar = lane >> 5;
    const int ci0 = blockIdx.x * 2, mt0 = blockIdx.y * 4, split = blockIdx.z;
    const int s_beg = split * a.per_split, s_end = min(a.nslice, s_beg + a.per_split);
    const int nst = s_end - s_beg;

    f32x16 acc[2][2];
#pragma unroll
    for (int i = 0; i < 2; ++i)
#pragma unroll
        for (int j = 0; j < 2; ++j)
#pragma unroll
            for (int q = 0; q < 16; ++q) acc[i][j][q] = 0.f;

    for (int e = tid; e < 2 * kBUF; e += 256) wl[e] = 0.f;

    if (nst > 0) {
        const lds_float* bb[2][2][4];
#pragma unroll
        for (int tn = 0; tn < 2; ++tn) {
            const int tap = tn * 32 + r, kd = tap >> 4, kh = (tap >> 2) & 3, kw = tap & 3;
            const int lb = wn * k4CH + kd * k4PLANE + kh * k4ROW + (kw & 1) * k4HALF + (kw >> 1) + kpar;
#pragma unroll
            for (int b = 0; b < 2; ++b)
#pragma unroll
                for (int od = 0; od < 4; ++od) {
                    bb[b][tn][od] = wl + b * kBUF + lb + od * (2 * k4PLANE);
                    pin_vgpr(bb[b][tn][od]);
                }
        }
        unsigned voff[4];
        lds_float* sdst[4];
#pragma unroll
        for (int f = 0; f < 4; ++f) {
            const int e = tid + 256 * f, c = e >> 9, idx = e & 511;
            const int id = idx >> 6, ih = (idx >> 3) & 7, iw = idx & 7;
            voff[f] = (ci0 + c) < a.Cin ? (unsigned)e * 4u : kBufOutside;
            sdst[f] = wl + c * k4CH + (id + 1) * k4PLANE + (ih + 1) * k4ROW + ((iw + 1) & 1) * k4HALF + ((iw + 1) >> 1);
            pin_vgpr(voff[f]);
            pin_vgpr(sdst[f]);
        }
        __amdgpu_buffer_rsrc_t ares[2];
#pragma unroll
        for (int t = 0; t < 2; ++t) ares[t] = make_rsrc(a.ap + ((long)(mt0 + wm * 2 + t) * a.nslice + s_beg) * 8 * 64);
        const unsigned avoff = lane * 16;
        const long slice_floats = (long)a.g.Cx * 512;
        const float* xb = a.x + (long)s_beg * slice_floats + (long)ci0 * 512;
        const int G = nst * 8;
        constexpr int kRing = 8;
        float fv[4];
        __syncthreads();
        {
            const __amdgpu_buffer_rsrc_t xres = make_rsrc(xb);
#pragma unroll
            for (int f = 0; f < 4; ++f) fv[f] = buf_load(xres, voff[f], 0);
        }
        float4 aring[kRing][2];
#pragma unroll
        for (int u = 0; u < kRing; ++u)
#pragma unroll
            for (int t = 0; t < 2; ++t) aring[u][t] = buf_load4(ares[t], avoff, (unsigned)(u < G ? u : G - 1) * 1024u);
#pragma unroll
        for (int f = 0; f < 4; ++f) *sdst[f] = fv[f];
        __syncthreads();

        auto stage = [&](auto tag, int st) {
            constexpr int CUR = decltype(tag)::value, NXT = CUR ^ 1;
            const int snext = st + 1 < nst ? st + 1 : st;
            const __amdgpu_buffer_rsrc_t xres = make_rsrc(xb + (long)snext * slice_floats);
            float bq[2][4];
#pragma unroll
            for (int tn = 0; tn < 2; ++tn) {
                const lds_float* hb = bb[CUR][tn][0];
                bq[tn][0] = hb[0];
                bq[tn][1] = hb[2];
                bq[tn][2] = hb[2 * k4ROW];
                bq[tn][3] = hb[2 * k4ROW + 2];
            }
            __builtin_amdgcn_sched_barrier(0);
#pragma unroll
            for (int gq = 0; gq < 8; ++gq) {
                float4 a_cur[2];
#pragma unroll
                for (int t = 0; t < 2; ++t) a_cur[t] = aring[gq][t];
                int gi = (st + 1) * 8 + gq;
                gi = gi < G ? gi : G - 1;
#pragma unroll
                for (int t = 0; t < 2; ++t) aring[gq][t] = buf_load4(ares[t], avoff, (unsigned)gi * 1024u);
                float b[2][4];
#pragma unroll
                for (int tn = 0; tn < 2; ++tn)
#pragma unroll
                    for (int j = 0; j < 4; ++j) b[tn][j] = bq[tn][j];
                if (gq + 1 < 8) {
#pragma unroll
                    for (int tn = 0; tn < 2; ++tn) {
                        const lds_float* hb = bb[CUR][tn][(gq + 1) >> 1] + ((gq + 1) & 1) * (4 * k4ROW);
                        bq[tn][0] = hb[0];
                        bq[tn][1] = hb[2];
                        bq[tn][2] = hb[2 * k4ROW];
                        bq[tn][3] = hb[2 * k4ROW + 2];
                    }
                }
                if (gq < 4) fv[gq] = buf_load(xres, voff[gq], 0);
                else sdst[gq - 4][NXT * kBUF] = fv[gq - 4];
                __builtin_amdgcn_sched_barrier(0);
#pragma unroll
                for (int j = 0; j < 4; ++j) {
                    const float a0 = j == 0 ? a_cur[0].x : (j == 1 ? a_cur[0].y : (j == 2 ? a_cur[0].z : a_cur[0].w));
                    const float a1 = j == 0 ? a_cur[1].x : (j == 1 ? a_cur[1].y : (j == 2 ? a_cur[1].z : a_cur[1].w));
                    acc[0][0] = __builtin_amdgcn_mfma_f32_32x32x2f32(a0, b[0][j], acc[0][0], 0, 0, 0);
                    acc[1][0] = __builtin_amdgcn_mfma_f32_32x32x2f32(a1, b[0][j], acc[1][0], 0, 0, 0);
                    acc[0][1] = __builtin_amdgcn_mfma_f32_32x32x2f32(a0, b[1][j], acc[0][1], 0, 0, 0);
                    acc[1][1] = __builtin_amdgcn_mfma_f32_32x32x2f32(a1, b[1][j], acc[1][1], 0, 0, 0);
                }
                __builtin_amdgcn_sched_barrier(0);
            }
            __syncthreads();
        };
        for (int st = 0; st + 1 < nst; st += 2) {
            stage(IntTag<0>(), st);
            stage(IntTag<1>(), st + 1);
        }
        if (nst & 1) stage(IntTag<0>(), nst - 1);
    }

    float* out = a.ws + (long)split * a.Cout * a.ldw;
#pragma unroll
    for (int tn = 0; tn < 2; ++tn) {
        const int col = wn * 64 + tn * 32 + r;
        const int ci = ci0 + (col >> 6);
        if (ci >= a.Cin) continue;
        const long cbase = (long)ci * 64 + (col & 63);
#pragma unroll
        for (int t = 0; t < 2; ++t) {
#pragma unroll
            for (int q = 0; q < 16; ++q) {
                const int co = (mt0 + wm * 2 + t) * 32 + (q & 3) + 8 * (q >> 2) + 4 * kpar;
                if (co < a.Cout) out[(long)co * a.ldw + cbase] = acc[t][tn][q];
            }
        }
    }
}

__global__ void __launch_bounds__(256) wgrad_halo_finalize_kernel(const float* __restrict__ ws, float* __restrict__ dw,
                                                                  int Cout, int ncol, long ldw, int nsplit) {
    const long total = (long)Cout * ncol, total4 = total >> 2;
    for (long e4 = (long)blockIdx.x * 256 + threadIdx.x; e4 < total4; e4 += (long)gridDim.x * 256) {
        const f32x4* p = reinterpret_cast<const f32x4*>(ws) + e4;
        f32x4 v = {0.f, 0.f, 0.f, 0.f};
        int s = 0;
        for (; s + 3 < nsplit; s += 4) {
            const f32x4 a0 = p[(long)s * total4], a1 = p[(long)(s + 1) * total4], a2 = p[(long)(s + 2) * total4],
                        a3 = p[(long)(s + 3) * total4];
            v += a0;
            v += a1;
            v += a2;
            v += a3;
        }
        for (; s < nsplit; ++s) v += p[(long)s * total4];
        const long e = e4 << 2;
        const long co = e / ncol, c = e - co * ncol;
        *reinterpret_cast<f32x4*>(dw + co * ldw + c) = v;
    }
}

static bool wgrad_mode4(const ConvGeom& g) { return g.OD == 4 && g.OH == 4 && g.OW == 4; }

static bool wgrad_rows64(const ConvGeom& g, int Cin, int Cout) {
    return !wgrad_mode4(g) && Cout <= 64 && Cin >= 4 && Cin % 4 == 0;
}
static void wgrad_halo_plan(int batch, const ConvGeom& g, int Cin, int Cout, int& nslice, int& nsplit, int& mtiles) {
    nslice = wgrad_mode4(g) ? batch : batch * g.OD * (g.OH / 8) * (g.OW / 8);
    const bool rows64 = wgrad_rows64(g, Cin, Cout);
    mtiles = rows64 ? (Cout + 63) / 64 : (Cout + 127) / 128;
    const int ntiles = (rows64 ? Cin / 4 : (Cin + 1) / 2) * mtiles;
    nsplit = (512 + ntiles - 1) / ntiles;
    if (nsplit > nslice / 4) nsplit = nslice / 4 > 0 ? nslice / 4 : 1;
    if (nsplit < 1) nsplit = 1;
}

size_t halo_wgrad_workspace_bytes(int batch, int Cin, int Cout, int OD, int OH, int OW) {
    if ((OH % 8 != 0 || OW % 8 != 0) && !(OD == 4 && OH == 4 && OW == 4)) return 0;
    ConvGeom g;
    g.OD = OD;
    g.OH = OH;
    g.OW = OW;
    int nslice, nsplit, mtiles;
    g.ID = 2 * OD;
    g.IH = 2 * OH;
    g.IW = 2 * OW;
    wgrad_halo_plan(batch, g, Cin, Cout, nslice, nsplit, mtiles);
    const size_t pack = (size_t)mtiles * 4 * nslice * 8 * 64 * sizeof(float4);
    const size_t part = (size_t)nsplit * Cout * Cin * 64 * sizeof(float);
    return pack + part + 256;
}

int halo_wgrad_dy_image_plan(int batch, int Cin, int Cout, const ConvGeom& g, size_t workspace_bytes, int* mt_total, long* nslice_out) {
    const bool mode4 = wgrad_mode4(g);
    if (!(mode4 || (g.OD == 8 && g.OH == 8 && g.OW == 8)) || Cout % 128 != 0 || Cin < 2) return 0;
    if ((long)batch * g.Cx * g.ID * g.IH * g.IW >= (1L << 31) || (long)2 * g.ID * g.IH * g.IW * 4 >= (1L << 26)) return 0;
    int nslice, nsplit, mtiles;
    wgrad_halo_plan(batch, g, Cin, Cout, nslice, nsplit, mtiles);
    const int ntiles = ((Cin + 1) / 2) * mtiles;
    if (Cout <= 64 || (long)ntiles * nsplit < 384) return 0;
    if (workspace_bytes < halo_wgrad_workspace_bytes(batch, Cin, Cout, g.OD, g.OH, g.OW)) return 0;
    *mt_total = mtiles * 4;
    *nslice_out = nslice;
    return 1;
}

__global__ void __launch_bounds__(256) act_bwd_pack8_kernel(const float* __restrict__ y, const float* __restrict__ dy,
                                                            float* __restrict__ dz, float* __restrict__ rowsum,
                                                            float4* __restrict__ ap, long rows, int C, long nslice, int act, float slope) {
    const long row = (long)blockIdx.x * 4 + (threadIdx.x >> 6);
    if (row >= rows) return;
    const int lane = threadIdx.x & 63;
    const long base = row * 512 + lane * 8;
    const f32x4 y0 = *reinterpret_cast<const f32x4*>(y + base), y1 = *reinterpret_cast<const f32x4*>(y + base + 4);
    const f32x4 g0 = *reinterpret_cast<const f32x4*>(dy + base), g1 = *reinterpret_cast<const f32x4*>(dy + base + 4);
    f32x4 z0, z1;
#pragma unroll
    for (int j = 0; j < 4; ++j) {
        z0[j] = act == SG_ACT_LEAKY ? (y0[j] > 0.f ? g0[j] : g0[j] * slope) : (y0[j] > 0.f ? g0[j] : 0.f);
        z1[j] = act == SG_ACT_LEAKY ? (y1[j] > 0.f ? g1[j] : g1[j] * slope) : (y1[j] > 0.f ? g1[j] : 0.f);
    }
    *reinterpret_cast<f32x4*>(dz + base) = z0;
    *reinterpret_cast<f32x4*>(dz + base + 4) = z1;
    const float s = sg_wave_sum(((z0[0] + z0[1]) + (z0[2] + z0[3])) + ((z1[0] + z1[1]) + (z1[2] + z1[3])));
    if (lane == 0) rowsum[row] = s;
    const long n = row / C;
    const int co = (int)(row - n * C), mt = co >> 5, r = co & 31, od = lane >> 3, oh = lane & 7;
    const long e = (((long)mt * nslice + n * 8 + od) * 8 + oh) * 64 + r;
    ap[e] = make_float4(z0[0], z0[2], z1[0], z1[2]);
    ap[e + 32] = make_float4(z0[1], z0[3], z1[1], z1[3]);
}
int halo_act_bwd_pack8_launch(const float* y, const float* dy, float* dz, float* rowsum, void* ap, long rows, int C, long nslice,
                              int act, float slope, hipStream_t stream) {
    hipLaunchKernelGGL(act_bwd_pack8_kernel, dim3((unsigned)((rows + 3) / 4)), dim3(256), 0, stream, y, dy, dz, rowsum, (float4*)ap,
                       rows, C, nslice, act, slope);
    return 1;
}

int halo_wgrad_try(const float* dy, const float* x, float* dw, int batch, int Cin, int Cin_total, const ConvGeom& g, int Cout,
                   void* workspace, size_t workspace_bytes, hipStream_t stream, int force, bool dy_packed) {
    const bool mode4 = wgrad_mode4(g);
    if ((!mode4 && (g.OW % 8 != 0 || g.OH % 8 != 0)) || Cin < 2 || Cout < 32) return 0;
    if ((long)batch * g.Cx * g.ID * g.IH * g.IW >= (1L << 31)) return 0;
    if ((long)2 * g.ID * g.IH * g.IW * 4 >= (1L << 26)) return 0;
    int nslice, nsplit, mtiles;
    wgrad_halo_plan(batch, g, Cin, Cout, nslice, nsplit, mtiles);
    const bool rows64 = wgrad_rows64(g, Cin, Cout) && (long)4 * g.ID * g.IH * g.IW * 4 < (1L << 26);
    if (wgrad_rows64(g, Cin, Cout) && !rows64) return 0;
    const int ntiles = (rows64 ? Cin / 4 : (Cin + 1) / 2) * mtiles;
    if (!force && ((Cout <= 64 && !rows64) || (long)ntiles * nsplit < 384)) return 0;
    const size_t need = halo_wgrad_workspace_bytes(batch, Cin, Cout, g.OD, g.OH, g.OW);
    if (!workspace || workspace_bytes < need) return 0;
    const int per_split = (nslice + nsplit - 1) / nsplit;
    nsplit = (nslice + per_split - 1) / per_split;

    const FastDiv dntw(mode4 ? 1 : g.OW / 8), dnth(mode4 ? 1 : g.OH / 8), dOD(g.OD);
    float4* ap = (float4*)workspace;
    const size_t pack_floats4 = (size_t)mtiles * 4 * nslice * 8 * 64;
    float* part = (float*)(ap + pack_floats4);
    if (!dy_packed) {
        int blocks = (int)((pack_floats4 + 255) / 256);
        if (blocks > 8192) blocks = 8192;
        if (mode4)
            hipLaunchKernelGGL(pack_wgrad_dy4_kernel, dim3(blocks), dim3(256), 0, stream, dy, ap, Cout, mtiles * 4, nslice);
        else
            hipLaunchKernelGGL(pack_wgrad_dy_kernel, dim3(blocks), dim3(256), 0, stream, dy, ap, g, Cout, rows64 ? mtiles * 2 : mtiles * 4,
                               nslice, dntw, dnth, dOD);
    }
    HaloWgradArgs a;
    a.ap = ap;
    a.x = x;
    a.g = g;
    a.Cin = Cin;
    a.Cout = Cout;
    a.nslice = nslice;
    a.per_split = per_split;
    a.mt_total = rows64 ? mtiles * 2 : mtiles * 4;
    a.dntw = dntw;
    a.dnth = dnth;
    a.dOD = dOD;
    const bool direct = nsplit == 1;
    a.ws = direct ? dw : part;
    a.ldw = direct ? (long)Cin_total * 64 : (long)Cin * 64;
    if (mode4) {
        hipLaunchKernelGGL(conv_wgrad_halo4_kernel, dim3((Cin + 1) / 2, mtiles, nsplit), dim3(256),
                           (size_t)2 * 2 * k4CH * sizeof(float), stream, a);
    } else {
        if (rows64) {
            const size_t lds = (size_t)2 * 4 * kWHS * sizeof(float);
            hipLaunchKernelGGL(conv_wgrad_halo_kernel<4>, dim3(Cin / 4, mtiles, nsplit), dim3(256), lds, stream, a);
        } else {
            const size_t lds = (size_t)2 * 2 * kWHS * sizeof(float);
            hipLaunchKernelGGL(conv_wgrad_halo_kernel<2>, dim3((Cin + 1) / 2, mtiles, nsplit), dim3(256), lds, stream, a);
        }
    }
    if (!direct) {
        const long total = (long)Cout * Cin * 64;
        int fb = (int)((total / 4 + 255) / 256);
        if (fb > 2048) fb = 2048;
        hipLaunchKernelGGL(wgrad_halo_finalize_kernel, dim3(fb), dim3(256), 0, stream, (const float*)part, dw, Cout, Cin * 64,
                           (long)Cin_total * 64, nsplit);
    }
    return 1;
}

}
```

shapegan_amd/ops.py:

```python
import ctypes
import weakref

import torch
from torch.autograd import Function
from torch.autograd.function import once_differentiable

from . import lib as L
from .lib import ACT_LEAKY, ACT_NONE, ACT_RELU, ACT_SIGMOID, ACT_TANH, check, f32c, ptr, stream, workspace


def _lib():
    return L.load()


def conv_fwd_raw(x, w, bias, act=ACT_NONE, slope=0.0, keep=False):
    N, Cx, D, H, W = x.shape
    Co, Ct = w.shape[0], w.shape[1]
    if Cx > Ct:
        raise RuntimeError("conv: input has %d channels, weight expects %d" % (Cx, Ct))
    ptr(x)
    L.reset_call_state()
    y = torch.empty((N, Co, D // 2, H // 2, W // 2), dtype=torch.float32, device=x.device)
    lib = _lib()
    nb = lib.sg_conv3d_k4s2p1_fwd_workspace_bytes(N, Cx, Co, D // 2, H // 2, W // 2)
    if keep and Cx > 1 and x.is_cuda and L.writers_known(w) and not torch.cuda.is_current_stream_capturing():
        ws, unchanged = _KEPT.get(w, nb, (N, Cx, Ct, Cx, Co, D, H, W), kind=0)
        check(lib.sg_conv3d_k4s2p1_fwd_keep(ptr(x), ptr(w), ptr(bias), ptr(y), N, Cx, Ct, Cx, Co, D, H, W, act, slope, ptr(ws),
                                            ws.numel(), int(unchanged), stream()), "conv3d_fwd_keep")
        return y
    ws = workspace("splitk", nb, x.device) if nb else None
    check(lib.sg_conv3d_k4s2p1_fwd(ptr(x), ptr(w), ptr(bias), ptr(y), N, Cx, Ct, Cx, Co, D, H, W, act, slope, ptr(ws),
                                   ws.numel() if ws is not None else 0, stream()), "conv3d_fwd")
    return y


def conv_fwd_impl_raw(x, w, bias, act, slope, impl, debug=0):
    N, Cx, D, H, W = x.shape
    Co, Ct = w.shape[0], w.shape[1]
    y = torch.empty((N, Co, D // 2, H // 2, W // 2), dtype=torch.float32, device=x.device)
    lib = _lib()
    nb = max(lib.sg_conv3d_k4s2p1_fwd_workspace_bytes(N, Cx, Co, D // 2, H // 2, W // 2), 1 << 20)
    ws = workspace("splitk", nb, x.device)
    check(lib.sg_conv3d_k4s2p1_fwd_impl(ptr(x), ptr(w), ptr(bias), ptr(y), N, Cx, Ct, Cx, Co, D, H, W, act, slope,
                                        ptr(ws), ws.numel(), impl, debug, stream()), "conv3d_fwd_impl")
    return y


class _KeptWeightImages(object):

    def __init__(self, cap=64):
        self.cap, self.entries, self.groups, self.layouts = cap, {}, {}, {}

    def _key(self, w, kind, dims, nbytes):
        if w.device.type != "cuda":
            return dims
        q = (kind, dims, int(nbytes))
        key = self.layouts.get(q)
        if key is None:
            if len(self.layouts) > 4096:
                self.layouts.clear()
            layout = _lib().sg_conv3d_k4s2p1_image_layout(kind, (ctypes.c_int * 8)(*[int(d) for d in dims]), int(nbytes))
            key = self.layouts[q] = ("layout", layout) if layout else dims
        return key

    def _ident(self, w, kind):
        return (w.device.index, stream(), w.data_ptr(), kind)

    def _state(self, w, shape_key):
        return (w._version, L.param_epoch_of(w), shape_key)

    def get(self, w, nbytes, shape_key, kind=1):
        ident = self._ident(w, kind)
        ent = self.entries.pop(ident, None)
        if ent is None or ent[0].numel() < nbytes or ent[2]() is not w:
            ent = [torch.empty(max(int(nbytes), 256), dtype=torch.uint8, device=w.device), None, weakref.ref(w), None]
        state = self._state(w, self._key(w, kind, shape_key, ent[0].numel()))
        unchanged = ent[1] == state
        if not unchanged:
            unchanged = self._pack_group(w, kind, ent, shape_key)
        ent[1], ent[3] = state, shape_key
        self.entries[ident] = ent
        while len(self.entries) > self.cap:
            self.entries.pop(next(iter(self.entries)))
        return ent[0], unchanged

    def _pack_group(self, w, kind, ent, shape_key):
        group = self.groups.get(id(w))
        if group is None or group[1]() is not w:
            return False
        jobs = [(w, kind, ent, shape_key)]
        for ref in group[0]:
            v = ref()
            if v is None or v.device != w.device:
                continue
            for k2 in (0, 1):
                if v is w and k2 == kind:
                    continue
                e2 = self.entries.get(self._ident(v, k2))
                if e2 is None or e2[2]() is not v or e2[1] is None:
                    continue
                if e2[1] != self._state(v, e2[1][2]):
                    jobs.append((v, k2, e2, e2[3]))
        if len(jobs) < 2:
            return False
        jobs = jobs[:8]
        n = len(jobs)
        kinds = (ctypes.c_int * n)(*[j[1] for j in jobs])
        wptr = (ctypes.c_void_p * n)(*[j[0].data_ptr() for j in jobs])
        wsp = (ctypes.c_void_p * n)(*[j[2][0].data_ptr() for j in jobs])
        wsb = (ctypes.c_size_t * n)(*[j[2][0].numel() for j in jobs])
        dims = (ctypes.c_int * (8 * n))(*[int(d) for j in jobs for d in j[3]])
        served = (ctypes.c_int * n)()
        L.note_device(w)
        check(_lib().sg_conv3d_k4s2p1_pack_images(n, kinds, wptr, wsp, wsb, dims, served, stream()), "conv3d_pack_images")
        for j, ok in zip(jobs[1:], list(served)[1:]):
            j[2][1] = self._state(j[0], self._key(j[0], j[1], j[3], j[2][0].numel())) if ok else None
        return bool(served[0])

    def register_group(self, weights):
        refs = [weakref.ref(w) for w in weights]
        for w in weights:
            self.groups[id(w)] = (refs, weakref.ref(w))


_KEPT = _KeptWeightImages()


def invalidate_weight_images():
    L.bump_param_epoch()


def register_pack_group(weights):
    _KEPT.register_group(list(weights))


def conv_dgrad_raw(dy, w, bias, cin, act=ACT_NONE, slope=0.0, keep=False, out=None):
    N, Co, OD, OH, OW = dy.shape
    Ct = w.shape[1]
    if w.shape[0] != Co or cin > Ct:
        raise RuntimeError("conv dgrad: shape mismatch")
    shape = (N, cin, 2 * OD, 2 * OH, 2 * OW)
    if out is not None:
        if tuple(out.shape) != shape or out.dtype != torch.float32 or not out.is_contiguous() or out.device != dy.device:
            raise RuntimeError("conv dgrad: `out` must be a contiguous fp32 tensor of shape %s on %s" % (shape, dy.device))
        dx = out
    else:
        dx = torch.empty(shape, dtype=torch.float32, device=dy.device)
    lib = _lib()
    nb = lib.sg_conv3d_k4s2p1_dgrad_workspace_bytes_for(N, cin, Co, OD, OH, OW)
    if keep and cin > 1 and dy.is_cuda and L.writers_known(w) and not torch.cuda.is_current_stream_capturing():
        ws, unchanged = _KEPT.get(w, nb, (N, cin, Ct, cin, Co, 2 * OD, 2 * OH, 2 * OW), kind=1)
        check(lib.sg_conv3d_k4s2p1_dgrad_keep(ptr(dy), ptr(w), ptr(bias), ptr(dx), N, cin, Ct, cin, Co, 2 * OD, 2 * OH, 2 * OW,
                                              act, slope, ptr(ws), ws.numel(), int(unchanged), stream()), "conv3d_dgrad_keep")
        return dx
    ws = workspace("dgrad", nb, dy.device)
    check(lib.sg_conv3d_k4s2p1_dgrad(ptr(dy), ptr(w), ptr(bias), ptr(dx), N, cin, Ct, cin, Co, 2 * OD, 2 * OH, 2 * OW,
                                     act, slope, ptr(ws), ws.numel(), stream()), "conv3d_dgrad")
    return dx


def conv_dgrad_halo_raw(dy, w, bias, cin, act=ACT_NONE, slope=0.0, impl=1):
    N, Co, OD, OH, OW = dy.shape
    Ct = w.shape[1]
    dx = torch.empty((N, cin, 2 * OD, 2 * OH, 2 * OW), dtype=torch.float32, device=dy.device)
    lib = _lib()
    ws = workspace("dgrad", lib.sg_conv3d_k4s2p1_dgrad_workspace_bytes(Co, cin), dy.device)
    check(lib.sg_conv3d_k4s2p1_dgrad_impl(ptr(dy), ptr(w), ptr(bias), ptr(dx), N, cin, Ct, cin, Co, 2 * OD, 2 * OH,
                                          2 * OW, act, slope, ptr(ws), ws.numel(), impl, stream()), "conv3d_dgrad_impl")
    return dx


_WGRAD_WS_CAP = 256 << 20


def _param_grad_out(param, shape, device):
    dst = L.grad_destination(param, shape) if param is not None else None
    return dst if dst is not None else torch.empty(shape, dtype=torch.float32, device=device)


def conv_wgrad_raw(dy, x, ct, out=None):
    N, Co, OD, OH, OW = dy.shape
    Cx = x.shape[1]
    if x.shape[0] != N or x.shape[2] != 2 * OD:
        raise RuntimeError("conv wgrad: shape mismatch")
    if out is not None:
        dw = out
        if Cx < ct:
            dw.zero_()
    elif Cx < ct:
        dw = torch.zeros((Co, ct, 4, 4, 4), dtype=torch.float32, device=dy.device)
    else:
        dw = torch.empty((Co, ct, 4, 4, 4), dtype=torch.float32, device=dy.device)
    lib = _lib()
    nb = min(lib.sg_conv3d_k4s2p1_wgrad_workspace_bytes(N, Cx, Co, OD, OH, OW), _WGRAD_WS_CAP)
    ws = workspace("splitk", nb, dy.device)
    check(lib.sg_conv3d_k4s2p1_wgrad(ptr(dy), ptr(x), ptr(dw), N, Cx, ct, Cx, Co, 2 * OD, 2 * OH, 2 * OW, ptr(ws),
                                     ws.numel(), stream()), "conv3d_wgrad")
    return dw


def _wgrad_dy_image(N, Cx, Co, O, device):
    if device.type != "cuda":
        return None
    lib = _lib()
    nb = min(lib.sg_conv3d_k4s2p1_wgrad_workspace_bytes(N, Cx, Co, O, O, O), _WGRAD_WS_CAP)
    ws = workspace("splitk", nb, device)
    mt, ns = ctypes.c_int(0), ctypes.c_long(0)
    if not lib.sg_conv3d_k4s2p1_wgrad_dy_image(N, Cx, Co, O, O, O, ws.numel(), ctypes.byref(mt), ctypes.byref(ns)):
        return None
    return ws, mt.value, ns.value


def conv_wgrad_prepacked_raw(dy, x, ct, ws, out=None):
    N, Co = dy.shape[0], dy.shape[1]
    Cx = x.shape[1]
    dw = out if out is not None else torch.empty((Co, ct, 4, 4, 4), dtype=torch.float32, device=dy.device)
    if Cx < ct:
        raise RuntimeError("conv_wgrad_prepacked: partial input channels are not served")
    check(_lib().sg_conv3d_k4s2p1_wgrad_prepacked(ptr(dy), ptr(x), ptr(dw), N, Cx, ct, Cx, Co, x.shape[2], x.shape[3], x.shape[4],
                                                  ptr(ws), ws.numel(), stream()), "conv3d_wgrad_prepacked")
    return dw


def act_bwd_rowsum_pack8_raw(y, dy, act, slope, ws, nslice, gb_out=None):
    y, dy = f32c(y), f32c(dy)
    N, C = y.shape[0], y.shape[1]
    lib = _lib()
    dz = torch.empty_like(y)
    rows = torch.empty(N * C, dtype=torch.float32, device=y.device)
    check(lib.sg_act_bwd_rowsum_pack8(ptr(y), ptr(dy), ptr(dz), ptr(rows), ptr(ws), N, C, nslice, act, slope, stream()),
          "act_bwd_rowsum_pack8")
    gb = torch.empty(C, dtype=torch.float32, device=y.device) if gb_out is None else gb_out
    check(lib.sg_colsum(ptr(rows), ptr(gb), N, C, C, stream()), "colsum")
    return dz, gb


def conv_wgrad_act_raw(dy, y, x, act, slope, dw_out=None, db_out=None):
    N, Co, OD, OH, OW = dy.shape
    Cx = x.shape[1]
    dw = dw_out if dw_out is not None else torch.empty((Co, Cx, 4, 4, 4), dtype=torch.float32, device=dy.device)
    db = db_out if db_out is not None else torch.empty(Co, dtype=torch.float32, device=dy.device)
    lib = _lib()
    nb = min(lib.sg_conv3d_k4s2p1_wgrad_workspace_bytes(N, Cx, Co, OD, OH, OW), _WGRAD_WS_CAP)
    ws = workspace("splitk", nb, dy.device)
    check(lib.sg_conv3d_k4s2p1_wgrad_act(ptr(dy), ptr(y), ptr(x), ptr(dw), ptr(db), N, Cx, Cx, Cx, Co, 2 * OD, 2 * OH, 2 * OW, act,
                                         slope, ptr(ws), ws.numel(), stream()), "conv3d_wgrad_act")
    return dw, db


def _wgrad_act_served(x, w, y, act):
    lib = _lib()
    N, Cx, Co = x.shape[0], x.shape[1], w.shape[0]
    if not lib.sg_conv3d_k4s2p1_wgrad_act_eligible(N, Cx, Co, y.shape[2], y.shape[3], y.shape[4], act):
        return False
    return lib.sg_conv3d_k4s2p1_wgrad_workspace_bytes(N, Cx, Co, y.shape[2], y.shape[3], y.shape[4]) <= _WGRAD_WS_CAP


def conv_wgrad_halo_raw(dy, x, ct):
    N, Co, OD, OH, OW = dy.shape
    Cx = x.shape[1]
    dw = torch.zeros((Co, ct, 4, 4, 4), dtype=torch.float32, device=dy.device)
    lib = _lib()
    ws = workspace("splitk", lib.sg_conv3d_k4s2p1_wgrad_workspace_bytes(N, Cx, Co, OD, OH, OW), dy.device)
    check(lib.sg_conv3d_k4s2p1_wgrad_impl(ptr(dy), ptr(x), ptr(dw), N, Cx, ct, Cx, Co, 2 * OD, 2 * OH, 2 * OW, ptr(ws),
                                          ws.numel(), 1, stream()), "conv3d_wgrad_impl")
    return dw


def gemm_raw(a, ta, b, tb, bias_j=None, bias_shift=0, act=ACT_NONE, slope=0.0, out=None, a_off=0, b_off=0, M=None,
             N=None, K=None, lda=None, ldb=None, ldc=None, c_off=0):
    lda = a.shape[-1] if lda is None else lda
    ldb = b.shape[-1] if ldb is None else ldb
    if M is None:
        M = a.shape[1] if ta else a.shape[0]
    if K is None:
        K = a.shape[0] if ta else a.shape[1]
    if N is None:
        N = b.shape[0] if tb else b.shape[1]
    sai, sak = (1, lda) if ta else (lda, 1)
    sbk, sbj = (1, ldb) if tb else (ldb, 1)
    if out is None:
        out = torch.empty((M, N), dtype=torch.float32, device=a.device)
    ldc = out.shape[-1] if ldc is None else ldc
    lib = _lib()
    nb = min(lib.sg_gemm_workspace_bytes(M, N), _WGRAD_WS_CAP)
    ws = workspace("splitk", nb, a.device)
    check(lib.sg_gemm(ptr(a) + 4 * a_off, sai, sak, ptr(b) + 4 * b_off, sbk, sbj, ptr(out) + 4 * c_off, ldc, 1, None,
                      ptr(bias_j), bias_shift, M, N, K, act, slope, ptr(ws), ws.numel(), stream()), "gemm")
    return out


def gemm_nt_raw(a, b, out, M, N, K, lda, ldb, ldc, a_off=0, b_off=0, c_off=0):
    lib = _lib()
    ws = workspace("gemm_nt", lib.sg_gemm_nt_workspace_bytes(M, N, K), a.device)
    check(lib.sg_gemm_nt(ptr(a) + 4 * a_off, lda, ptr(b) + 4 * b_off, ldb, ptr(out) + 4 * c_off, ldc, M, N, K, ptr(ws),
                         ws.numel(), stream()), "gemm_nt")
    return out


def act_bwd_raw(y, dy, act, slope):
    dx = torch.empty_like(y)
    check(_lib().sg_act_bwd(ptr(y), ptr(dy), ptr(dx), y.numel(), act, slope, stream()), "act_bwd")
    return dx


def act_bwd_rowsum_raw(y, dy, act, slope, gb_out=None):
    y, dy = f32c(y), f32c(dy)
    N, C = y.shape[0], y.shape[1]
    S = y.numel() // (N * C)
    lib = _lib()
    dz = torch.empty_like(y)
    rows = torch.empty(N * C, dtype=torch.float32, device=y.device)
    check(lib.sg_act_bwd_rowsum(ptr(y), ptr(dy), ptr(dz), ptr(rows), N * C, S, act, slope, stream()), "act_bwd_rowsum")
    gb = torch.empty(C, dtype=torch.float32, device=y.device) if gb_out is None else gb_out
    check(lib.sg_colsum(ptr(rows), ptr(gb), N, C, C, stream()), "colsum")
    return dz, gb


def act_fwd_raw(x, act, slope):
    y = torch.empty_like(x)
    check(_lib().sg_act_fwd(ptr(x), ptr(y), x.numel(), act, slope, stream()), "act_fwd")
    return y


def channel_sum_raw(g, out=None):
    N, C = g.shape[0], g.shape[1]
    S = g.numel() // (N * C)
    lib = _lib()
    if out is None:
        out = torch.empty(C, dtype=torch.float32, device=g.device)
    if S == 1:
        check(lib.sg_colsum(ptr(g), ptr(out), N, C, C, stream()), "colsum")
        return out
    tmp = torch.empty(N * C, dtype=torch.float32, device=g.device)
    check(lib.sg_rowsum(ptr(g), ptr(tmp), N * C, S, S, stream()), "rowsum")
    check(lib.sg_colsum(ptr(tmp), ptr(out), N, C, C, stream()), "colsum")
    return out


class ActBwd(Function):

    @staticmethod
    def forward(ctx, y, dy, act, slope):
        y, dy = f32c(y), f32c(dy)
        ctx.act, ctx.slope = act, slope
        ctx.save_for_backward(y)
        ctx.dy = dy if act in (ACT_TANH, ACT_SIGMOID) else None
        return act_bwd_raw(y, dy, act, slope)

    @staticmethod
    def backward(ctx, ggx):
        (y,) = ctx.saved_tensors
        g_dy = ActBwd.apply(y, ggx, ctx.act, ctx.slope) if ctx.needs_input_grad[1] else None
        g_y = None
        if ctx.needs_input_grad[0] and ctx.act in (ACT_TANH, ACT_SIGMOID):
            dy = ctx.dy
            g_y = torch.empty_like(y)
            check(_lib().sg_act_bwd_dy(ptr(y), ptr(f32c(dy.detach())), ptr(f32c(ggx.detach())), ptr(g_y), y.numel(), ctx.act,
                                       stream()), "act_bwd_dy")
        return g_y, g_dy, None, None


class Act(Function):

    @staticmethod
    def forward(ctx, x, act, slope):
        x = f32c(x)
        y = act_fwd_raw(x, act, slope)
        ctx.act, ctx.slope = act, slope
        ctx.save_for_backward(y)
        return y

    @staticmethod
    def backward(ctx, gy):
        (y,) = ctx.saved_tensors
        return ActBwd.apply(y, gy, ctx.act, ctx.slope), None, None


class ChannelSum(Function):
    @staticmethod
    def forward(ctx, g):
        g = f32c(g)
        ctx.shape = g.shape
        return channel_sum_raw(g)

    @staticmethod
    def backward(ctx, gg):
        shape = ctx.shape
        view = [1, shape[1]] + [1] * (len(shape) - 2)
        return gg.reshape(view).expand(shape)


class ConvFwd(Function):

    @staticmethod
    def forward(ctx, x, w, b, act, slope):
        x, w = f32c(x), f32c(w)
        y = conv_fwd_raw(x, w, b, act, slope, keep=True)
        ctx.act, ctx.slope, ctx.has_b = act, slope, b is not None
        ctx.save_for_backward(x, w, y if act != ACT_NONE else None, b)
        return y

    @staticmethod
    def backward(ctx, gy):
        x, w, y, b = ctx.saved_tensors
        gb = None
        want_b = ctx.has_b and ctx.needs_input_grad[2]
        plain = not torch.is_grad_enabled()
        if (ctx.act != ACT_NONE and want_b and plain and ctx.needs_input_grad[1] and not ctx.needs_input_grad[0]
                and w.shape[1] == x.shape[1] and _wgrad_act_served(x, w, y, ctx.act)):
            gw, gb = conv_wgrad_act_raw(f32c(gy), y, x, ctx.act, ctx.slope, L.grad_destination(w, w.shape),
                                        L.grad_destination(b, b.shape))
            return None, gw, gb, None, None
        image = None
        if (ctx.act in (ACT_LEAKY, ACT_RELU) and want_b and plain and ctx.needs_input_grad[1] and tuple(y.shape[2:]) == (8, 8, 8)
                and w.shape[1] == x.shape[1] and y.shape[1] % 128 == 0):
            image = _wgrad_dy_image(x.shape[0], x.shape[1], w.shape[0], 8, y.device)
        if image is not None:
            gz, gb = act_bwd_rowsum_pack8_raw(y, gy, ctx.act, ctx.slope, image[0], image[2], L.grad_destination(b, b.shape))
        elif ctx.act != ACT_NONE and want_b and plain and y.shape[2] * y.shape[3] * y.shape[4] >= 512:
            gz, gb = act_bwd_rowsum_raw(y, gy, ctx.act, ctx.slope, L.grad_destination(b, b.shape))
        else:
            gz = ActBwd.apply(y, gy, ctx.act, ctx.slope) if ctx.act != ACT_NONE else gy
        gx = None
        if ctx.needs_input_grad[0]:
            gx = conv_dgrad_raw(f32c(gz), w, None, x.shape[1], keep=True) if plain else ConvDgrad.apply(gz, w, None, x.shape[1], ACT_NONE, 0.0)
        gw = None
        if ctx.needs_input_grad[1]:
            if image is not None:
                gw = conv_wgrad_prepacked_raw(gz, x, w.shape[1], image[0], L.grad_destination(w, w.shape))
            else:
                gw = conv_wgrad_raw(f32c(gz), x, w.shape[1], L.grad_destination(w, w.shape)) if plain else ConvWgrad.apply(gz, x, w.shape[1])
        if want_b and gb is None:
            gb = channel_sum_raw(f32c(gz), L.grad_destination(b, b.shape)) if plain else ChannelSum.apply(gz)
        return gx, gw, gb, None, None


class ConvDgrad(Function):

    @staticmethod
    def forward(ctx, dy, w, b, cin, act, slope, keep=False):
        dy, w = f32c(dy), f32c(w)
        dx = conv_dgrad_raw(dy, w, b, cin, act, slope, keep)
        ctx.act, ctx.slope, ctx.has_b = act, slope, b is not None
        ctx.save_for_backward(dy, w, dx if act != ACT_NONE else None, b)
        return dx

    @staticmethod
    def backward(ctx, gdx):
        dy, w, dx, b = ctx.saved_tensors
        g_b = None
        want_b = ctx.has_b and ctx.needs_input_grad[2]
        plain = not torch.is_grad_enabled()
        if ctx.act != ACT_NONE and want_b and plain and dx.shape[2] * dx.shape[3] * dx.shape[4] >= 512:
            gz, g_b = act_bwd_rowsum_raw(dx, gdx, ctx.act, ctx.slope, L.grad_destination(b, b.shape))
        else:
            gz = ActBwd.apply(dx, gdx, ctx.act, ctx.slope) if ctx.act != ACT_NONE else gdx
        g_dy = ConvFwd.apply(gz, w, None, ACT_NONE, 0.0) if ctx.needs_input_grad[0] else None
        g_w = None
        if ctx.needs_input_grad[1]:
            g_w = conv_wgrad_raw(dy, f32c(gz), w.shape[1], L.grad_destination(w, w.shape)) if plain else ConvWgrad.apply(dy, gz, w.shape[1])
        if want_b and g_b is None:
            g_b = channel_sum_raw(f32c(gz), L.grad_destination(b, b.shape)) if plain else ChannelSum.apply(gz)
        return g_dy, g_w, g_b, None, None, None, None


class ConvWgrad(Function):

    @staticmethod
    def forward(ctx, dy, x, ct):
        dy, x = f32c(dy), f32c(x)
        ctx.save_for_backward(dy, x)
        return conv_wgrad_raw(dy, x, ct)

    @staticmethod
    def backward(ctx, gdw):
        dy, x = ctx.saved_tensors
        g_dy = ConvFwd.apply(x, gdw, None, ACT_NONE, 0.0) if ctx.needs_input_grad[0] else None
        g_x = ConvDgrad.apply(dy, gdw, None, x.shape[1], ACT_NONE, 0.0) if ctx.needs_input_grad[1] else None
        return g_dy, g_x, None


def conv3d_k4s2p1(x, w, b, act=ACT_NONE, slope=0.0):
    return ConvFwd.apply(x, w, b, act, slope)


def conv_transpose3d_k4s2p1(x, w, b, act=ACT_NONE, slope=0.0, out=None):
    if out is not None and not torch.is_grad_enabled():
        return conv_dgrad_raw(f32c(x), f32c(w), b, w.shape[1], act, slope, True, out)
    return ConvDgrad.apply(x, w, b, w.shape[1], act, slope, True)


def convT_to1_pre_eligible(N, C, D, H, W):
    return bool(_lib().sg_convT3d_k4s2p1_to1_pre_eligible(int(N), int(C), int(D), int(H), int(W)))


def convT_to1_pre_served(x, w):
    return (w.shape[1] == 1 and x.dim() == 5 and
            bool(_lib().sg_convT3d_k4s2p1_to1_pre_eligible(x.shape[0], x.shape[1], x.shape[2], x.shape[3], x.shape[4])))


def bn_train_stats_affine(x, gamma, beta, running_mean, running_var, num_batches_tracked, eps, momentum, groups=1):
    x = f32c(x)
    N, C = x.shape[0], x.shape[1]
    if N % groups:
        raise RuntimeError("bn_train_stats_affine: %d samples in %d groups" % (N, groups))
    S = x.numel() // (N * C)
    lib = _lib()
    mean = torch.empty((groups, C), dtype=torch.float32, device=x.device)
    invstd, scale, shift = torch.empty_like(mean), torch.empty_like(mean), torch.empty_like(mean)
    ws = workspace("bn", groups * lib.sg_bn_workspace_bytes(C), x.device)
    check(lib.sg_bn_train_stats_grouped(ptr(x), ptr(gamma), ptr(beta), ptr(mean), ptr(invstd), ptr(running_mean), ptr(running_var),
                                        ptr(num_batches_tracked), ptr(scale), ptr(shift), groups, N // groups, C, S, eps, momentum,
                                        ptr(ws), ws.numel(), stream()), "bn_train_stats")
    return (scale, shift) if groups > 1 else (scale[0], shift[0])


def bn_train_fwd_grouped_raw(x, gamma, beta, running_mean, running_var, num_batches_tracked, eps, momentum, act, slope, groups):
    x = f32c(x)
    N, C = x.shape[0], x.shape[1]
    if N % groups:
        raise RuntimeError("bn_train_fwd_grouped: %d samples in %d groups" % (N, groups))
    S = x.numel() // (N * C)
    lib = _lib()
    y = torch.empty_like(x)
    mean = torch.empty((groups, C), dtype=torch.float32, device=x.device)
    invstd = torch.empty_like(mean)
    ws = workspace("bn", groups * lib.sg_bn_workspace_bytes(C), x.device)
    check(lib.sg_bn_train_fwd_grouped(ptr(x), ptr(gamma), ptr(beta), ptr(y), ptr(mean), ptr(invstd), ptr(running_mean),
                                      ptr(running_var), ptr(num_batches_tracked), groups, N // groups, C, S, eps, momentum, act,
                                      slope, ptr(ws), ws.numel(), stream()), "bn_train_fwd_grouped")
    return y


def conv_transpose3d_to1_pre_raw(x, scale, shift, in_act, in_slope, w, b, act=ACT_NONE, slope=0.0, out=None, outs=None, form=0):
    x, w = f32c(x), f32c(w)
    N, C, D, H, W = x.shape
    if outs is not None:
        groups = len(outs)
        per = N // groups
        want = (per, 1, 2 * D, 2 * H, 2 * W)
        stride = (outs[1].data_ptr() - outs[0].data_ptr()) // 4 if groups > 1 else per * 8 * D * H * W
        for g, o in enumerate(outs):
            if (tuple(o.shape) != want or o.dtype != torch.float32 or not o.is_contiguous() or o.device != x.device
                    or o.data_ptr() != outs[0].data_ptr() + 4 * stride * g):
                raise RuntimeError("conv_transpose3d_to1_pre: `outs` must be equally spaced contiguous fp32 tensors of shape %s" % (want,))
        if N % groups or tuple(scale.shape) != (groups, C) or stride < per * 8 * D * H * W:
            raise RuntimeError("conv_transpose3d_to1_pre: %d samples, %d groups, scale %s" % (N, groups, tuple(scale.shape)))
        check(_lib().sg_convT3d_k4s2p1_to1_pre_grouped(ptr(x), ptr(w), ptr(b), ptr(outs[0]), ptr(scale), ptr(shift), in_act, in_slope,
                                                       N, C, D, H, W, act, slope, per, stride, stream()), "convT3d_to1_pre_grouped")
        return outs
    shape = (N, 1, 2 * D, 2 * H, 2 * W)
    if out is not None:
        if tuple(out.shape) != shape or out.dtype != torch.float32 or not out.is_contiguous() or out.device != x.device:
            raise RuntimeError("conv_transpose3d_to1_pre: `out` must be a contiguous fp32 tensor of shape %s on %s" % (shape, x.device))
        y = out
    else:
        y = torch.empty(shape, dtype=torch.float32, device=x.device)
    if form:
        args = (ptr(x), ptr(w), ptr(b), ptr(y), ptr(scale), ptr(shift), in_act, in_slope, N, C, D, H, W, act, slope, int(form), stream())
        L.reset_call_state()
        if not x.is_cuda:
            raise RuntimeError("conv_transpose3d_to1_pre: kernel forms exist on the GPU only")
        check(L._load_hip().sg_convT3d_k4s2p1_to1_pre_impl(*args), "convT3d_to1_pre_impl")
        return y
    check(_lib().sg_convT3d_k4s2p1_to1_pre(ptr(x), ptr(w), ptr(b), ptr(y), ptr(scale), ptr(shift), in_act, in_slope, N, C, D, H, W,
                                           act, slope, stream()), "convT3d_to1_pre")
    return y
# ... 1498 lines not shown
```

Before: 60.00 steps/s.

## Skip zero-padding depth slabs in halo conv forward, dgrad and wgrad kernels

Specializes the LDS-halo forward, dgrad and wgrad conv kernels by boundary class, so blocks at the first or last depth slab skip the kernel taps and MFMA work that only touch zero padding. Block-to-depth mapping is rotated by batch index so boundary blocks spread across the grid. Forward remaps the weight ring to 6 of 8 taps for boundary slabs. The cost is more template instantiations, with added code size and register pressure, and more complex indexing. Debug flags can disable the skip and the rotation.

```diff
diff --git a/shapegan_amd/csrc/conv3d.hip b/shapegan_amd/csrc/conv3d.hip
--- a/shapegan_amd/csrc/conv3d.hip
+++ b/shapegan_amd/csrc/conv3d.hip
@@ -746,8 +746,8 @@
 int sg_conv3d_k4s2p1_dgrad_impl(const float* dy, const float* w, const float* bias, float* dx, int batch, int Cin,
                                 int Cin_total, int Cx, int Cout, int ID, int IH, int IW, int act, float slope,
                                 void* workspace, size_t workspace_bytes, int impl, hipStream_t stream) {
-    SG_CHECK_ARG(dy && w && dx && batch > 0 && Cin > 0 && Cin <= Cin_total && Cin <= Cx && Cout > 0 && (impl & 1) &&
-                 (impl == 1 || impl == 3 || impl == 9 || impl == 17 || impl == 33));
+    SG_CHECK_ARG(dy && w && dx && batch > 0 && Cin > 0 && Cin <= Cin_total && Cin <= Cx && Cout > 0 && (impl & 1) && impl < 512 &&
+                 ((impl & 63) == 1 || (impl & 63) == 3 || (impl & 63) == 9 || (impl & 63) == 17 || (impl & 63) == 33));
     ConvGeom g;
     if (make_geom(g, ID, IH, IW, Cx, Cout)) SG_FAIL(SG_ERR_ARG, "sg_conv3d_k4s2p1_dgrad_impl: bad spatial dims");
     if (check_sizes(g, batch, "sg_conv3d_k4s2p1_dgrad_impl")) return SG_ERR_ARG;
@@ -761,11 +761,11 @@
 int sg_conv3d_k4s2p1_wgrad_impl(const float* dy, const float* x, float* dw, int batch, int Cin, int Cin_total, int Cx,
                                 int Cout, int ID, int IH, int IW, void* workspace, size_t workspace_bytes, int impl,
                                 hipStream_t stream) {
-    SG_CHECK_ARG(dy && x && dw && batch > 0 && Cin > 0 && Cin <= Cin_total && Cin <= Cx && Cout > 0 && impl == 1);
+    SG_CHECK_ARG(dy && x && dw && batch > 0 && Cin > 0 && Cin <= Cin_total && Cin <= Cx && Cout > 0 && (impl == 1 || impl == 65));
     ConvGeom g;
     if (make_geom(g, ID, IH, IW, Cx, Cout)) SG_FAIL(SG_ERR_ARG, "sg_conv3d_k4s2p1_wgrad_impl: bad spatial dims");
     if (check_sizes(g, batch, "sg_conv3d_k4s2p1_wgrad_impl")) return SG_ERR_ARG;
-    const int rc = halo_wgrad_try(dy, x, dw, batch, Cin, Cin_total, g, Cout, workspace, workspace_bytes, stream, 1);
+    const int rc = halo_wgrad_try(dy, x, dw, batch, Cin, Cin_total, g, Cout, workspace, workspace_bytes, stream, impl);
     if (rc != 1) SG_FAIL(SG_ERR_ARG, "sg_conv3d_k4s2p1_wgrad_impl: shape not eligible for the LDS-halo kernel");
     SG_CHECK_LAUNCH();
     return SG_OK;
diff --git a/shapegan_amd/csrc/conv3d_halo.hip b/shapegan_amd/csrc/conv3d_halo.hip
--- a/shapegan_amd/csrc/conv3d_halo.hip
+++ b/shapegan_amd/csrc/conv3d_halo.hip
@@ -30,6 +30,7 @@
     int csplit;
     float* partial;
     long npos;
+    int flags;
 };
 
 __global__ void __launch_bounds__(256) pack_fwd_weights_kernel(const float* __restrict__ w, float4* __restrict__ wp,
@@ -51,8 +52,10 @@
     }
 }
 
-template <int TN, int NW>
-__global__ void __launch_bounds__(NW * 64) conv_fwd_halo_kernel(HaloFwdArgs a) {
+template <int TN, int NW, int SLAB>
+__device__ __forceinline__ void conv_fwd_halo_body(const HaloFwdArgs& a, const uint32_t twi, const uint32_t thi, const uint32_t od,
+                                                   const uint32_t n) {
+    constexpr int J0 = SLAB == 1 ? 2 : 0, NJ = SLAB ? 6 : 8, NG = kCC * NJ;
     constexpr int kFR = NW * 2;
     constexpr int kNF = (kHD * kHH + kFR - 1) / kFR;
     constexpr int WN = 2 / TN;
@@ -62,10 +65,6 @@
     extern __shared__ __attribute__((aligned(16))) float halo[];
     lds_float* const hl = (lds_float*)halo;
 
-    uint32_t twi, thi, od, n, q1, q2;
-    a.dntw.divmod(blockIdx.x, q1, twi);
-    a.dnth.divmod(q1, q2, thi);
-    a.dOD.divmod(q2, n, od);
     const int oh0 = thi * 8, ow0 = twi * 8;
     const int co0 = blockIdx.y * ROWS;
 
@@ -125,7 +124,8 @@
         for (int f = 0; f < kNF; ++f) fv[c][f] = buf_load(xres, goff[f], c * chan_bytes);
     float4 aring[kRing];
 #pragma unroll
-    for (int u = 0; u < kRing; ++u) aring[u] = buf_load4(wres, wvoff, (unsigned)(u < G ? u : G - 1) * 1024u);
+    for (int u = 0; u < kRing; ++u)
+        aring[u] = buf_load4(wres, wvoff, (unsigned)((u / NJ) * 8 + J0 + u % NJ) * 1024u);
 #pragma unroll
     for (int c = 0; c < kCC; ++c)
 #pragma unroll
@@ -133,17 +133,18 @@
     __syncthreads();
 
     const int nstage = a.Cin / kCC;
-    int gbase = kRing;
 
     auto stage = [&](auto tag, int s) {
         constexpr int CUR = decltype(tag)::value, NXT = CUR ^ 1;
+        static_assert(NG % kRing == 0, "ring slots must line up at the stage boundary");
+        const int gst = s * (8 * kCC);
         int cnext = (s + 1) * kCC;
         cnext = cnext > a.Cin - kCC ? a.Cin - kCC : cnext;
         const unsigned xs = (unsigned)cnext * chan_bytes;
         float bq[TN][4];
 #pragma unroll
         for (int u = 0; u < TN; ++u) {
-            const lds_float* hb = bb[CUR][0][0] + u * kTNOFF;
+            const lds_float* hb = bb[CUR][0][J0 >> 1] + u * kTNOFF;
             bq[u][0] = hb[0];
             bq[u][1] = hb[1];
             bq[u][2] = hb[kROWH];
@@ -153,19 +154,20 @@
 #pragma unroll
         for (int ci = 0; ci < kCC; ++ci) {
 #pragma unroll
-            for (int j = 0; j < 8; ++j) {
-                const float4 a_cur = aring[(ci * 8 + j) % kRing];
-                int gi = gbase + ci * 8 + j;
+            for (int jj = 0; jj < NJ; ++jj) {
+                const int t = ci * NJ + jj;
+                const float4 a_cur = aring[t % kRing];
+                int gi = gst + ((t + kRing) / NJ) * 8 + J0 + (t + kRing) % NJ;
                 gi = gi < G ? gi : G - 1;
-                if (!(SG_ABLATE & 4)) aring[(ci * 8 + j) % kRing] = buf_load4(wres, wvoff, (unsigned)gi * 1024u);
+                if (!(SG_ABLATE & 4)) aring[t % kRing] = buf_load4(wres, wvoff, (unsigned)gi * 1024u);
                 {
                     constexpr int NE = kCC * kNF;
-                    const int gidx = ci * 8 + j;
+                    const int gidx = t;
 #pragma unroll
                     for (int e = 0; e < NE; ++e) {
                         const int c = e / kNF, f = e % kNF;
-                        if (e * 24 / NE + 8 == gidx && !(SG_ABLATE & 2)) sdst[f][NXT * kBUF + c * kHS] = fv[c][f];
-                        if (e * 24 / NE == gidx && !(SG_ABLATE & 3)) fv[c][f] = buf_load(xres, goff[f], xs + c * chan_bytes);
+                        if (e * (NG - 8) / NE + 8 == gidx && !(SG_ABLATE & 2)) sdst[f][NXT * kBUF + c * kHS] = fv[c][f];
+                        if (e * (NG - 8) / NE == gidx && !(SG_ABLATE & 3)) fv[c][f] = buf_load(xres, goff[f], xs + c * chan_bytes);
                     }
                 }
                 float b[TN][4];
@@ -173,8 +175,8 @@
                 for (int u = 0; u < TN; ++u)
 #pragma unroll
                     for (int k = 0; k < 4; ++k) b[u][k] = bq[u][k];
-                if (!(ci == kCC - 1 && j == 7) && !(SG_ABLATE & 16)) {
-                    const int jn = (j + 1) & 7, cin = ci + ((j + 1) >> 3);
+                if (t + 1 < NG && !(SG_ABLATE & 16)) {
+                    const int jn = J0 + (t + 1) % NJ, cin = (t + 1) / NJ;
                     const lds_float* hb = bb[CUR][cin][jn >> 1] + (2 * (jn & 1)) * kROWH;
 #pragma unroll
                     for (int u = 0; u < TN; ++u) {
@@ -195,7 +197,6 @@
                 __builtin_amdgcn_sched_barrier(0);
             }
         }
-        gbase += 8 * kCC;
         __syncthreads();
     };
     for (int s = 0; s + 1 < nstage; s += 2) {
@@ -221,6 +222,28 @@
             if (co < a.Cout) yo[(long)co * O3] = sg_apply_act(acc[u][q] + bv[q], a.act, a.slope);
         }
     }
+}
+
+template <int TN, int NW>
+__global__ void __launch_bounds__(NW * 64) conv_fwd_halo_kernel(HaloFwdArgs a) {
+    uint32_t twi, thi, od, n, q1, q2;
+    a.dntw.divmod(blockIdx.x, q1, twi);
+    a.dnth.divmod(q1, q2, thi);
+    a.dOD.divmod(q2, n, od);
+    if (!(a.flags & 2)) {
+        uint32_t nq, nr;
+        a.dOD.divmod(n, nq, nr);
+        od += nr;
+        od -= od >= (uint32_t)a.g.OD ? (uint32_t)a.g.OD : 0u;
+    }
+    const int slab = __builtin_amdgcn_readfirstlane(
+        (a.flags & 1) || a.g.OD == 1 ? 0 : (od == 0 ? 1 : ((int)od == a.g.OD - 1 ? 2 : 0)));
+    if (slab == 0)
+        conv_fwd_halo_body<TN, NW, 0>(a, twi, thi, od, n);
+    else if (slab == 1)
+        conv_fwd_halo_body<TN, NW, 1>(a, twi, thi, od, n);
+    else
+        conv_fwd_halo_body<TN, NW, 2>(a, twi, thi, od, n);
 }
 
 constexpr int k4HALF = 5, k4ROW = 10, k4PLANE = 104, k4CH = 10 * k4PLANE;
@@ -402,6 +425,7 @@
         a.act = act;
         a.slope = slope;
         a.csplit = csplit;
+        a.flags = 0;
         a.partial = reinterpret_cast<float*>(static_cast<char*>(workspace) + halo_fwd_workspace_bytes(Cin, Cout));
         a.npos = (long)batch * 64;
         const size_t lds4 = (size_t)2 * k4BUF * sizeof(float);
@@ -458,6 +482,10 @@
     a.dOD = FastDiv(g.OD);
     a.act = act;
     a.slope = slope;
+    a.csplit = 1;
+    a.partial = nullptr;
+    a.npos = 0;
+    a.flags = (debug >> 8) & 3;
     dim3 grid((unsigned)tiles, mtiles);
     if (rows == 128 && variant == 2)
         hipLaunchKernelGGL((conv_fwd_halo_kernel<1, 8>), grid, dim3(512), lds, stream, a);
@@ -491,6 +519,7 @@
     FastDiv dntw, dnth, dntd;
     int act;
     float slope;
+    int flags;
 };
 
 __global__ void __launch_bounds__(256) pack_dgrad_frag_kernel(const float* __restrict__ w, float4* __restrict__ wp,
@@ -573,21 +602,17 @@
     return jobs.n;
 }
 
-template <int MODE, bool R32>
-__device__ __forceinline__ void conv_dgrad_halo_body(HaloDgradArgs a) {
+template <int MODE, bool R32, int CLS = 0>
+__device__ __forceinline__ void conv_dgrad_halo_body(const HaloDgradArgs& a, const uint32_t twi, const uint32_t thi, const uint32_t tdi,
+                                                     const uint32_t n) {
     constexpr int NTN = R32 ? 1 : 2;
     constexpr int kDCC = 16, kDNF = 16, kDBUF = kDNF * 256;
     using BX = DBox<MODE>;
     constexpr int kDB = BX::CH;
+    constexpr bool SW = MODE == 0 && !R32;
+    constexpr int TNOFF = SW ? BX::WNOFF : BX::TNOFF, WNOFF = SW ? BX::TNOFF : BX::WNOFF;
     extern __shared__ __attribute__((aligned(16))) float box[];
-    uint32_t twi = 0, thi = 0, tdi = 0, n, q1, q2;
-    if (MODE == 0) {
-        a.dntw.divmod(blockIdx.x, q1, twi);
-        a.dnth.divmod(q1, q2, thi);
-        a.dntd.divmod(q2, n, tdi);
-    } else {
-        n = blockIdx.x * 2;
-    }
+    static_assert(SW || CLS == 0, "only the 64-row MODE 0 form skips");
     const int qd0 = tdi * 2, qh0 = thi * 8, qw0 = twi * 8;
     const int ci0 = blockIdx.y * (R32 ? 32 : 64);
 
@@ -596,7 +621,7 @@
     const int wm = R32 ? 0 : wave >> 1, wn = wave & 1, r = lane & 31, kpar = lane >> 5;
     const int tnf = R32 ? wave >> 1 : 0;
     const int lpart = MODE == 0 ? (r >> 3) * BX::BW + (r & 7) : (r >> 4) * BX::PL + ((r >> 2) & 3) * BX::BW + (r & 3);
-    const int lanebase = wn * BX::WNOFF + tnf * BX::TNOFF + lpart + 1 - kpar;
+    const int lanebase = wn * WNOFF + tnf * TNOFF + lpart + 1 - kpar;
 
     f32x16 acc[NTN];
 #pragma unroll
@@ -663,8 +688,8 @@
     for (int tn = 0; tn < NTN; ++tn) {
         int qd, qh, qw;
         if (MODE == 0) {
-            qd = qd0 + wn;
-            qh = qh0 + (tnf + tn) * 4 + (r >> 3);
+            qd = qd0 + (SW ? tn : wn);
+            qh = qh0 + (SW ? wn : tnf + tn) * 4 + (r >> 3);
             qw = qw0 + (r & 7);
         } else {
             qd = 2 * (tnf + tn) + (r >> 4);
@@ -750,16 +775,16 @@
 
     constexpr int O00 = BX::PL + BX::BW, O01 = BX::PL, O10 = BX::BW, O11 = 0;
     const int nstage = a.Cout / kDCC;
-    auto stage = [&](auto tag, unsigned dys, unsigned wnext) __attribute__((always_inline)) {
-        constexpr int CUR = decltype(tag)::value, NXT = CUR ^ 1;
+    auto stage = [&](auto tag, auto sktag, unsigned dys, unsigned wnext) __attribute__((always_inline)) {
+        constexpr int CUR = decltype(tag)::value, NXT = CUR ^ 1, SK = decltype(sktag)::value;
+        constexpr int OJ[4] = {O00, O01, O10, O11};
+        auto skipped = [](int tn, int j) constexpr { return (SK == 1 && tn == 0 && j >= 2) || (SK == 2 && tn == 1 && j < 2); };
         float bq[NTN][4];
 #pragma unroll
         for (int tn = 0; tn < NTN; ++tn) {
-            const lds_float* hb = bb[CUR][0] + tn * BX::TNOFF;
-            bq[tn][0] = hb[O00];
-            bq[tn][1] = hb[O01];
-            bq[tn][2] = hb[O10];
-            bq[tn][3] = hb[O11];
+            const lds_float* hb = bb[CUR][0] + tn * TNOFF;
+#pragma unroll
+            for (int j = 0; j < 4; ++j) bq[tn][j] = skipped(tn, j) ? 0.f : hb[OJ[j]];
         }
         __builtin_amdgcn_sched_barrier(0);
 #pragma unroll
@@ -775,11 +800,10 @@
             if (c + 1 < kDCC) {
 #pragma unroll
                 for (int tn = 0; tn < NTN; ++tn) {
-                    const lds_float* hb = bb[CUR][c + 1] + tn * BX::TNOFF;
-                    bq[tn][0] = hb[O00];
-                    bq[tn][1] = hb[O01];
-                    bq[tn][2] = hb[O10];
-                    bq[tn][3] = hb[O11];
+                    const lds_float* hb = bb[CUR][c + 1] + tn * TNOFF;
+#pragma unroll
+                    for (int j = 0; j < 4; ++j)
+                        if (!skipped(tn, j)) bq[tn][j] = hb[OJ[j]];
                 }
             }
             if (c < kDCC / 2) {
@@ -794,35 +818,86 @@
 #pragma unroll
             for (int j = 0; j < 4; ++j)
 #pragma unroll
-                for (int tn = 0; tn < NTN; ++tn) acc[tn] = __builtin_amdgcn_mfma_f32_32x32x2f32(av[j], b[tn][j], acc[tn], 0, 0, 0);
+                for (int tn = 0; tn < NTN; ++tn)
+                    if (!skipped(tn, j)) acc[tn] = __builtin_amdgcn_mfma_f32_32x32x2f32(av[j], b[tn][j], acc[tn], 0, 0, 0);
             __builtin_amdgcn_sched_barrier(0);
         }
         wcur = wnext;
         __syncthreads();
     };
-    for (int par = par0; par < par_end; ++par) {
+    auto parity = [&](auto sktag, int par) __attribute__((always_inline)) {
         const bool more = par + 1 < par_end;
         const unsigned wlast = more ? (unsigned)(par + 1) * par_bytes : (unsigned)par * par_bytes + (unsigned)(nstage - 1) * kDCC * 1024u;
         const unsigned dlast = more ? 0u : (unsigned)(nstage - 1) * kDCC * chan_bytes;
         int s = 0;
         for (; s + 1 < nstage; s += 2) {
-            stage(IntTag<0>(), (unsigned)(s + 1) * kDCC * chan_bytes, wcur + kDCC * 1024u);
+            stage(IntTag<0>(), sktag, (unsigned)(s + 1) * kDCC * chan_bytes, wcur + kDCC * 1024u);
             const bool last = s + 2 == nstage;
             if (last && more) set_goff(par + 1);
-            stage(IntTag<1>(), last ? dlast : (unsigned)(s + 2) * kDCC * chan_bytes, last ? wlast : wcur + kDCC * 1024u);
-        }
-        if (s < nstage) stage(IntTag<0>(), dlast, wlast);
-        write_parity(par);
-    }
-}
-
+            stage(IntTag<1>(), sktag, last ? dlast : (unsigned)(s + 2) * kDCC * chan_bytes, last ? wlast : wcur + kDCC * 1024u);
+        }
+        if (s < nstage) stage(IntTag<0>(), sktag, dlast, wlast);
+    };
+    constexpr int SKLO = (CLS & 1) ? 1 : 0, SKHI = (CLS & 2) ? 2 : 0;
+    if constexpr (SKLO == SKHI) {
+        for (int par = par0; par < par_end; ++par) {
+            parity(IntTag<0>(), par);
+            write_parity(par);
+        }
+    } else {
+        const int mid = par_end < 4 ? par_end : (par0 > 4 ? par0 : 4);
+        for (int par = par0; par < mid; ++par) {
+            parity(IntTag<SKLO>(), par);
+            write_parity(par);
+        }
+        for (int par = mid; par < par_end; ++par) {
+            parity(IntTag<SKHI>(), par);
+            write_parity(par);
+        }
+    }
+}
+
+template <int MODE>
+__device__ __forceinline__ void dgrad_decode(const HaloDgradArgs& a, uint32_t& twi, uint32_t& thi, uint32_t& tdi, uint32_t& n) {
+    twi = thi = tdi = 0;
+    if (MODE == 0) {
+        uint32_t q1, q2;
+        a.dntw.divmod(blockIdx.x, q1, twi);
+        a.dnth.divmod(q1, q2, thi);
+        a.dntd.divmod(q2, n, tdi);
+    } else {
+        n = blockIdx.x * 2;
+    }
+}
 template <int MODE>
 __global__ void __launch_bounds__(256) conv_dgrad_halo_kernel(HaloDgradArgs a) {
-    conv_dgrad_halo_body<MODE, false>(a);
+    uint32_t twi, thi, tdi, n;
+    dgrad_decode<MODE>(a, twi, thi, tdi, n);
+    if constexpr (MODE == 0) {
+        if (!(a.flags & 2)) {
+            uint32_t nq, nr;
+            a.dntd.divmod(n, nq, nr);
+            tdi += nr;
+            tdi -= tdi >= a.dntd.d ? a.dntd.d : 0u;
+        }
+        const int cls = __builtin_amdgcn_readfirstlane((a.flags & 1) ? 0 : (tdi == 0 ? 1 : 0) | (tdi + 1 == a.dntd.d ? 2 : 0));
+        if (cls == 0)
+            conv_dgrad_halo_body<0, false, 0>(a, twi, thi, tdi, n);
+        else if (cls == 1)
+            conv_dgrad_halo_body<0, false, 1>(a, twi, thi, tdi, n);
+        else if (cls == 2)
+            conv_dgrad_halo_body<0, false, 2>(a, twi, thi, tdi, n);
+        else
+            conv_dgrad_halo_body<0, false, 3>(a, twi, thi, tdi, n);
+    } else {
+        conv_dgrad_halo_body<MODE, false>(a, twi, thi, tdi, n);
+    }
 }
 template <int MODE>
 __global__ void __launch_bounds__(256) conv_dgrad_halo32_kernel(HaloDgradArgs a) {
-    conv_dgrad_halo_body<MODE, true>(a);
+    uint32_t twi, thi, tdi, n;
+    dgrad_decode<MODE>(a, twi, thi, tdi, n);
+    conv_dgrad_halo_body<MODE, true>(a, twi, thi, tdi, n);
 }
 
 size_t halo_dgrad_workspace_bytes(int Cin, int Cout) { return (size_t)8 * ((Cin + 63) / 64) * 64 * Cout * 8 * sizeof(float); }
@@ -866,9 +941,10 @@
     a.dntd = FastDiv(ntd);
     a.act = act;
     a.slope = slope;
+    a.flags = (force >> 6) & 3;
     int ppw = 8;
     while (ppw > 1 && (tiles * mtiles * (8 / ppw) < 512 || (force & 2) || (Cout / 16) % 2 != 0)) ppw >>= 1;
-    if ((force >> 2) && (Cout / 16) % 2 == 0) ppw = force >> 2;
+    if (((force >> 2) & 15) && (Cout / 16) % 2 == 0) ppw = (force >> 2) & 15;
     if ((long)8 * mtiles * 2 * Cout * 1024 >= (long)kBufRange) return 0;
     a.ppw = ppw;
     size_t lds = (size_t)2 * 16 * 256 * sizeof(float);
@@ -877,7 +953,7 @@
         const long cost2 = ((wgs + 511) / 512) * 2, cost3 = ((wgs + 767) / 768) * 3;
         if (cost2 <= cost3) lds = 56 * 1024;
     }
-    const bool r32 = Cin <= 32 || tiles * mtiles * (8 / ppw) < 256;
+    const bool r32 = Cin <= 32 || (!(force & 256) && tiles * mtiles * (8 / ppw) < 256);
     const dim3 grid((unsigned)tiles, r32 ? (unsigned)((Cin + 31) / 32) : (unsigned)mtiles, 8 / ppw);
     if (mode1 && r32)
         hipLaunchKernelGGL((conv_dgrad_halo32_kernel<1>), grid, dim3(256), lds, stream, a);
@@ -902,6 +978,7 @@
     int Cin, Cout, nslice, per_split, mt_total;
     long ldw;
     FastDiv dntw, dnth, dOD;
+    int flags;
 };
 
 __global__ void __launch_bounds__(256) pack_wgrad_dy_kernel(const float* __restrict__ dy, float4* __restrict__ ap,
@@ -929,8 +1006,182 @@
     }
 }
 
+constexpr int kWHS2 = kWHS + 16;
+constexpr int kWB2 = 2 * kWHS2;
+template <bool SAMPLES>
+__device__ __forceinline__ void conv_wgrad_halo_planes_body(const HaloWgradArgs& a) {
+    extern __shared__ __attribute__((aligned(16))) float wbox[];
+    const int tid = threadIdx.x, lane = tid & 63;
+    const int wave = __builtin_amdgcn_readfirstlane(tid >> 6);
+    const int r = lane & 31, kpar = lane >> 5;
+    const int ci0 = blockIdx.x * 2;
+    const int mt = blockIdx.y * 4 + wave;
+    const int split = blockIdx.z;
+    const int s_beg = split * a.per_split, s_end = min(a.nslice, s_beg + a.per_split);
+    const int lanebase = (r >> 4) * kWHS2 + ((r >> 2) & 3) * kROWH + (r & 1) * kHWH + ((r >> 1) & 1) + kpar;
+
+    f32x16 acc[4];
+#pragma unroll
+    for (int t = 0; t < 4; ++t)
+#pragma unroll
+        for (int q = 0; q < 16; ++q) acc[t][q] = 0.f;
+
+    const int I3 = a.g.ID * a.g.IH * a.g.IW;
+    const int fl_w = tid & 31, frow = tid >> 5;
+    const int lds_w = (fl_w & 1) * kHWH + (fl_w >> 1);
+    const int prow = (tid >> 1) % (kHD * kHH);
+    const int pad = (prow / kHH) * kWROWD + (prow % kHH) * kROWH + (tid & 1) * kHWH + (kHWH - 1);
+    lds_float* const wl = (lds_float*)wbox;
+    lds_float* sdst[kWNF / 2];
+    unsigned voff[kWNF], cls[kWNF];
+#pragma unroll
+    for (int f = 0; f < kWNF / 2; ++f) {
+        const int row = 8 * f + frow;
+        const int hd = row / kHH, hh = row - hd * kHH;
+        const bool inbox = fl_w < kHWF && row < kHD * kHH;
+        sdst[f] = wl + (inbox ? hd * kWROWD + hh * kROWH + lds_w : pad);
+        pin_vgpr(sdst[f]);
+#pragma unroll
+        for (int c = 0; c < 2; ++c) {
+            const bool ok = inbox && (ci0 + c) < a.Cin;
+            voff[c * (kWNF / 2) + f] = ok ? (unsigned)(c * I3 + (hd * a.g.IH + hh) * a.g.IW + fl_w) * 4u : kBufOutside;
+            cls[c * (kWNF / 2) + f] = (hd == 0 ? 1u << 26 : 0u) | (hd == kHD - 1 ? 1u << 27 : 0u) | (hh == 0 ? 1u << 28 : 0u) |
+                                      (hh == kHH - 1 ? 1u << 29 : 0u) | (fl_w == 0 ? 1u << 30 : 0u) |
+                                      (fl_w == kHWF - 1 ? 1u << 31 : 0u);
+            pin_vgpr(voff[c * (kWNF / 2) + f]);
+            pin_vgpr(cls[c * (kWNF / 2) + f]);
+        }
+    }
+    float fv[kWNF];
+    unsigned eoff[kWNF];
+    __amdgpu_buffer_rsrc_t xres;
+    const int ntw_ = (int)a.g.OW / 8, nth_ = (int)a.g.OH / 8;
+    auto copy_prepare = [&](int sl) __attribute__((always_inline)) {
+        uint32_t twi, thi, od, n, q1, q2;
+        a.dntw.divmod((uint32_t)sl, q1, twi);
+        a.dnth.divmod(q1, q2, thi);
+        a.dOD.divmod(q2, n, od);
+        const long origin = ((long)n * a.g.Cx + ci0) * I3 + ((2 * (long)od - 1) * a.g.IH + (16 * (long)thi - 1)) * a.g.IW +
+                            (16 * (long)twi - 1);
+        xres = __builtin_amdgcn_make_buffer_rsrc(const_cast<float*>(a.x + origin), 0, 1 << 26, 0x00020000);
+        const unsigned flags = (od == 0 ? 1u << 26 : 0u) | ((int)od == a.g.OD - 1 ? 1u << 27 : 0u) | (thi == 0 ? 1u << 28 : 0u) |
+                               ((int)thi == nth_ - 1 ? 1u << 29 : 0u) | (twi == 0 ? 1u << 30 : 0u) |
+                               ((int)twi == ntw_ - 1 ? 1u << 31 : 0u);
+#pragma unroll
+        for (int f = 0; f < kWNF; ++f) eoff[f] = (cls[f] & flags) | voff[f];
+    };
+
+    const int nst = s_end - s_beg;
+    constexpr int kRing = 8;
+    const int G = nst * 8;
+    if (nst > 0) {
+        const __amdgpu_buffer_rsrc_t ares = make_rsrc(a.ap + ((long)mt * a.nslice + s_beg) * 8 * 64);
+        const unsigned avoff = lane * 16;
+        const lds_float* bb[2];
+#pragma unroll
+        for (int b = 0; b < 2; ++b) {
+            bb[b] = wl + b * kWB2 + lanebase;
+            pin_vgpr(bb[b]);
+        }
+
+        copy_prepare(s_beg);
+#pragma unroll
+        for (int f = 0; f < kWNF; ++f) fv[f] = buf_load(xres, eoff[f], 0);
+        float4 aring[kRing];
+#pragma unroll
+        for (int u = 0; u < kRing; ++u) aring[u] = buf_load4(ares, avoff, (unsigned)(u < G ? u : G - 1) * 1024u);
+#pragma unroll
+        for (int f = 0; f < kWNF; ++f) sdst[f % (kWNF / 2)][(f / (kWNF / 2)) * kWHS2] = fv[f];
+        __syncthreads();
+
+        auto stage = [&](auto tag, auto stag, int st) __attribute__((always_inline)) {
+            constexpr int CUR = decltype(tag)::value, NXT = CUR ^ 1, SLAB = decltype(stag)::value;
+            constexpr int T0 = SLAB == 1 ? 1 : 0, T1 = SLAB == 2 ? 3 : 4;
+            const int snext = st + 1 < nst ? st + 1 : st;
+            float bq[4][4];
+#pragma unroll
+            for (int t = T0; t < T1; ++t)
+#pragma unroll
+                for (int j = 0; j < 4; ++j) bq[t][j] = bb[CUR][t * kWROWD + 2 * j];
+            copy_prepare(s_beg + snext);
+            __builtin_amdgcn_sched_barrier(0);
+#pragma unroll
+            for (int gq = 0; gq < 8; ++gq) {
+                const float4 a_cur = aring[gq];
+                int gi = (st + 1) * 8 + gq;
+                gi = gi < G ? gi : G - 1;
+                aring[gq] = buf_load4(ares, avoff, (unsigned)gi * 1024u);
+                float b[4][4];
+#pragma unroll
+                for (int t = T0; t < T1; ++t)
+#pragma unroll
+                    for (int j = 0; j < 4; ++j) b[t][j] = bq[t][j];
+                if (gq + 1 < 8) {
+#pragma unroll
+                    for (int t = T0; t < T1; ++t)
+#pragma unroll
+                        for (int j = 0; j < 4; ++j) bq[t][j] = bb[CUR][t * kWROWD + 2 * (gq + 1) * kROWH + 2 * j];
+                }
+#pragma unroll
+                for (int f = 0; f < kWNF; ++f) {
+                    if (f * 4 / kWNF == gq) fv[f] = buf_load(xres, eoff[f], 0);
+                    if (f * 4 / kWNF + 4 == gq) sdst[f % (kWNF / 2)][NXT * kWB2 + (f / (kWNF / 2)) * kWHS2] = fv[f];
+                }
+                __builtin_amdgcn_sched_barrier(0);
+                const float av[4] = {a_cur.x, a_cur.y, a_cur.z, a_cur.w};
+#pragma unroll
+                for (int j = 0; j < 4; ++j)
+#pragma unroll
+                    for (int t = T0; t < T1; ++t) acc[t] = __builtin_amdgcn_mfma_f32_32x32x2f32(av[j], b[t][j], acc[t], 0, 0, 0);
+                __builtin_amdgcn_sched_barrier(0);
+            }
+            __syncthreads();
+        };
+        if constexpr (SAMPLES) {
+            for (int st = 0; st < nst;) {
+                stage(IntTag<0>(), IntTag<1>(), st);
+                ++st;
+                for (int k = 2; k < a.g.OD; k += 2, st += 2) {
+                    stage(IntTag<1>(), IntTag<0>(), st);
+                    stage(IntTag<0>(), IntTag<0>(), st + 1);
+                }
+                stage(IntTag<1>(), IntTag<2>(), st);
+                ++st;
+            }
+        } else {
+            for (int st = 0; st + 1 < nst; st += 2) {
+                stage(IntTag<0>(), IntTag<0>(), st);
+                stage(IntTag<1>(), IntTag<0>(), st + 1);
+            }
+            if (nst & 1) stage(IntTag<0>(), IntTag<0>(), nst - 1);
+        }
+    }
+
+    float* out = a.ws + (long)split * a.Cout * a.ldw;
+    const int ci = ci0 + (r >> 4);
+    if (ci < a.Cin) {
+#pragma unroll
+        for (int t = 0; t < 4; ++t) {
+            const long cbase = (long)ci * 64 + t * 16 + (r & 15);
+#pragma unroll
+            for (int q = 0; q < 16; ++q) {
+                const int co = mt * 32 + (q & 3) + 8 * (q >> 2) + 4 * kpar;
+                if (co < a.Cout) out[(long)co * a.ldw + cbase] = acc[t][q];
+            }
+        }
+    }
+}
+
+
 template <int NCH>
 __global__ void __launch_bounds__(256) conv_wgrad_halo_kernel(HaloWgradArgs a) {
+    if constexpr (NCH == 2) {
+        if (a.flags & 1)
+            conv_wgrad_halo_planes_body<true>(a);
+        else
+            conv_wgrad_halo_planes_body<false>(a);
+        return;
+    }
     extern __shared__ __attribute__((aligned(16))) float wbox[];
     const int tid = threadIdx.x, lane = tid & 63;
     const int wave = __builtin_amdgcn_readfirstlane(tid >> 6);
@@ -1434,6 +1685,7 @@
     a.dntw = dntw;
     a.dnth = dnth;
     a.dOD = dOD;
+    a.flags = !(force & 64) && !mode4 && g.OH == 8 && g.OW == 8 && g.OD >= 2 && g.OD % 2 == 0 && per_split % g.OD == 0 ? 1 : 0;
     const bool direct = nsplit == 1;
     a.ws = direct ? dw : part;
     a.ldw = direct ? (long)Cin_total * 64 : (long)Cin * 64;
@@ -1445,7 +1697,7 @@
             const size_t lds = (size_t)2 * 4 * kWHS * sizeof(float);
             hipLaunchKernelGGL(conv_wgrad_halo_kernel<4>, dim3(Cin / 4, mtiles, nsplit), dim3(256), lds, stream, a);
         } else {
-            const size_t lds = (size_t)2 * 2 * kWHS * sizeof(float);
+            const size_t lds = (size_t)2 * kWB2 * sizeof(float);
             hipLaunchKernelGGL(conv_wgrad_halo_kernel<2>, dim3((Cin + 1) / 2, mtiles, nsplit), dim3(256), lds, stream, a);
         }
     }
diff --git a/shapegan_amd/ops.py b/shapegan_amd/ops.py
--- a/shapegan_amd/ops.py
+++ b/shapegan_amd/ops.py
@@ -32,6 +32,11 @@
     check(lib.sg_conv3d_k4s2p1_fwd(ptr(x), ptr(w), ptr(bias), ptr(y), N, Cx, Ct, Cx, Co, D, H, W, act, slope, ptr(ws),
                                    ws.numel() if ws is not None else 0, stream()), "conv3d_fwd")
     return y
+
+
+HALO_FWD_NO_SLAB_SKIP, HALO_FWD_NO_ROTATION = 256, 512
+HALO_DGRAD_NO_SLAB_SKIP, HALO_DGRAD_NO_ROTATION, HALO_DGRAD_ROWS64 = 64, 128, 256
+HALO_WGRAD_NO_SLAB_SKIP = 64
 
 
 def conv_fwd_impl_raw(x, w, bias, act, slope, impl, debug=0):
@@ -256,14 +261,14 @@
     return lib.sg_conv3d_k4s2p1_wgrad_workspace_bytes(N, Cx, Co, y.shape[2], y.shape[3], y.shape[4]) <= _WGRAD_WS_CAP
 
 
-def conv_wgrad_halo_raw(dy, x, ct):
+def conv_wgrad_halo_raw(dy, x, ct, impl=1):
     N, Co, OD, OH, OW = dy.shape
     Cx = x.shape[1]
     dw = torch.zeros((Co, ct, 4, 4, 4), dtype=torch.float32, device=dy.device)
     lib = _lib()
     ws = workspace("splitk", lib.sg_conv3d_k4s2p1_wgrad_workspace_bytes(N, Cx, Co, OD, OH, OW), dy.device)
     check(lib.sg_conv3d_k4s2p1_wgrad_impl(ptr(dy), ptr(x), ptr(dw), N, Cx, ct, Cx, Co, 2 * OD, 2 * OH, 2 * OW, ptr(ws),
-                                          ws.numel(), 1, stream()), "conv3d_wgrad_impl")
+                                          ws.numel(), impl, stream()), "conv3d_wgrad_impl")
     return dw
 
 
```

Measured after the change: 59.74 steps/s. Within noise of the previous version (-0.4%).
